# boolsi/boolsi

Measured on AMD Instinct MI355X. Metric: node-state-updates/s, higher is better.
Workload: dtype u32

## Files before the change

boolsi_amd/csrc/bsx_cascade.cpp:

```cpp
#include <cmath>
#include <cstdio>
#include <cstring>

#include "bsx_attract_host.h"

using namespace bsx;

namespace {
constexpr uint64_t kUnresCap = 1ull << 16;
constexpr uint64_t kNearBytes = 1ull << 32;
}

namespace bsx {

static int mirror_slots_for(bsx_handle h, uint32_t* slots_out) {
    const uint64_t entries = (h->cube_mirror ? 2 : 1) * h->journal_states;
    uint32_t slots = 64;
    while (slots < 2 * entries && slots < h->cache_lds_slots) slots *= 2;
    const size_t fixed = h->shmem + 32 + pool_extra_bytes(h->net.nw);
    while (slots < 4 * entries && slots < h->cache_lds_slots && fixed + (size_t)2 * slots * h->cache_stride <= 80 * 1024) slots *= 2;
    h->mirror_slots = *slots_out = std::min(slots, h->cache_lds_slots);
    if (h->knobs.debug) std::fprintf(stderr, "[bsx] mirror: %llu cycle states cached, %u slots\n", (unsigned long long)h->journal_states, *slots_out);
    return BSX_OK;
}

int lean_mirror_slots(bsx_handle h, uint32_t* slots_out, Totals* tot) {
    uint32_t ignored = 0;
    if (!slots_out) slots_out = &ignored;
    if (!h->journal_stale) return mirror_slots_for(h, slots_out);
    unsigned int known = 0;
    HIPCHK(h, hipMemcpy(&known, h->d_cc_count.p, sizeof(known), hipMemcpyDeviceToHost));
    if (tot) ++tot->syncs;
    known = std::min<unsigned int>(known, kCycleJournalCap);
    h->h_journal.resize(known);
    if (known) HIPCHK(h, hipMemcpy(h->h_journal.data(), h->d_cc_journal.p, known * sizeof(CycleRecord), hipMemcpyDeviceToHost));
    uint64_t states = 0;
    uint32_t taken = 0;
    for (const CycleRecord& r : h->h_journal) {
        if (taken >= (uint32_t)kTagAcc + kLdsAcc) break;
        if (!r.ready || r.length == 0 || r.length > kCycleCacheMaxLen) continue;
        states += r.length;
        ++taken;
    }
    h->journal_states = states;
    h->journal_stale = false;
    return mirror_slots_for(h, slots_out);
}

int ensure_mirror_image(bsx_handle h, AttractParams& P, size_t shmem) {
    if (!h->knobs.mirror_image) { P.mirror_image = nullptr; P.mirror_out = nullptr; return BSX_OK; }
    const size_t words = 4 + (size_t)P.cc.lds_slots * (h->cache_stride / 4);
    if (h->image_n != h->h_journal.size() || h->image_slots != P.cc.lds_slots || h->d_mirror.n < words) {
        HIPCHK(h, h->d_mirror.reserve(words));
        AttractParams B = P;
        B.count = 0;
        B.level_in = nullptr;
        B.mirror_image = nullptr;
        B.mirror_out = h->d_mirror.p;
        HIPCHK(h, launch_attract_pool((int)h->net.nw, (int)h->net.k_mux, h->lut_mode, dim3(1), shmem, h->stream, B));
        h->image_n = h->h_journal.size();
        h->image_slots = P.cc.lds_slots;
    }
    P.mirror_image = h->d_mirror.p;
    P.mirror_out = nullptr;
    return BSX_OK;
}

}

namespace {

int order_cube_digits(bsx_handle h, Cube& c) {
    const uint32_t r = (uint32_t)c.rel.size();
    if (r < 2 || r > 64 || !h->knobs.cube_order) return BSX_OK;
    uint64_t need = 0;
    for (uint32_t q = 0; q < r; ++q) need |= 1ull << c.rel[q];
    if (need & ~h->life_valid) {
        LifetimeParams L{};
        L.net = h->net;
        for (int w = 0; w < kMaxW32; ++w) { L.fixmask[w] = h->sp.fixmask[w]; L.fixval[w] = h->sp.fixval[w]; L.base[w] = c.base[w]; L.free_mask[w] = c.free_mask[w]; }
        L.n_digits = r;
        for (uint32_t q = 0; q < r; ++q) L.node[q] = h->model.any[c.rel[q]];
        HIPCHK(h, h->d_life.reserve(64));
        HIPCHK(h, hipMemsetAsync(h->d_life.p, 0, 64 * sizeof(uint32_t), h->stream));
        L.out = h->d_life.p;
        HIPCHK(h, launch_digit_lifetimes((int)h->net.nw, (int)h->net.k_mux, h->lut_mode, h->shmem, h->stream, L));
        uint32_t measured[64];
        HIPCHK(h, hipMemcpyAsync(measured, h->d_life.p, sizeof(measured), hipMemcpyDeviceToHost, h->stream));
        HIPCHK(h, hipStreamSynchronize(h->stream));
        for (uint32_t q = 0; q < r; ++q) h->life_cache[c.rel[q]] = measured[q];
        h->life_valid |= need;
    }
    uint32_t life[64];
    for (uint32_t q = 0; q < r; ++q) life[q] = h->life_cache[c.rel[q]];
    std::vector<uint32_t> idx(r);
    for (uint32_t q = 0; q < r; ++q) idx[q] = q;
    std::stable_sort(idx.begin(), idx.end(), [&](uint32_t x, uint32_t y) { return life[x] < life[y]; });
    std::vector<uint32_t> rel(r);
    for (uint32_t q = 0; q < r; ++q) rel[q] = c.rel[idx[q]];
    c.rel = rel;
    return BSX_OK;
}

int fetch_counters(bsx_handle h, uint32_t n_blocks) {
    if (!h->knobs.spin_wait) {
        HIPCHK(h, hipMemcpyAsync(h->h_ctr, h->d_ctr, sizeof(Counters) * n_blocks, hipMemcpyDeviceToHost, h->stream));
        HIPCHK(h, hipStreamSynchronize(h->stream));
        return BSX_OK;
    }
    const uint32_t seq = ++h->flag_seq ? h->flag_seq : ++h->flag_seq;
    HIPCHK(h, launch_publish(reinterpret_cast<const uint32_t*>(h->d_ctr), reinterpret_cast<uint32_t*>(h->h_ctr),
                             (uint32_t)(sizeof(Counters) / 4 * n_blocks), const_cast<uint32_t*>(h->h_flag), seq,
                             reinterpret_cast<unsigned int*>(reinterpret_cast<char*>(h->d_level) + kPublishTicketOffset), h->stream));
    uint32_t polls = 0;
    while (__atomic_load_n(h->h_flag, __ATOMIC_ACQUIRE) != seq) {
        __builtin_ia32_pause();
        if ((++polls & 0xFFFFu) == 0) {
            const hipError_t q = hipStreamQuery(h->stream);
            if (q == hipSuccess) {
                if (__atomic_load_n(h->h_flag, __ATOMIC_ACQUIRE) == seq) break;
                return fail(h, BSX_ERR_HIP, "the cascade finished without publishing its counters");
            }
            if (q != hipErrorNotReady) { h->error = std::string("hipStreamQuery: ") + hipGetErrorString(q); return BSX_ERR_HIP; }
        }
    }
    return BSX_OK;
}

CascadeShape cascade_shape(bsx_handle h, const CascadeEnv& env) {
    CascadeShape sh{};
    sh.tp = h->sp.tp_origin;
    sh.cap_rel = env.max_t == BSX_T_INF ? BSX_T_INF : env.max_t - sh.tp;
    sh.cap_rel32 = (sh.cap_rel == BSX_T_INF || sh.cap_rel >= (kStepLimit / 4)) ? 0xFFFFFFFFu : (uint32_t)sh.cap_rel;
    sh.fast_steps = (uint32_t)std::min<uint64_t>((uint64_t)sh.cap_rel32 + 1, std::min<uint32_t>(kFastStepsMax, std::max(192u, 4 * h->fast_steps)));
    uint32_t max_depth = h->knobs.cube_depth ? h->knobs.cube_depth : 8;
    if (h->plan.cube_depth_cap) max_depth = std::min(max_depth, h->plan.cube_depth_cap);
    if (sh.tp) max_depth = (uint32_t)std::min<uint64_t>(max_depth, sh.tp);
    sh.max_depth = std::max(1u, std::min(max_depth, sh.fast_steps > 1 ? sh.fast_steps - 1 : 1u));
    sh.forced_depth = h->knobs.cube_depth != 0;
    return sh;
}

struct ChainLevel {
    uint32_t depth = 0, k_bits = 0, r_here = 0, unit_shift = 0;
    bool per_parent = false;
    Cube cube;
};
struct Chain {
    Cube c1;
    std::vector<uint64_t> rel_mask;
    std::vector<ChainLevel> lv;
    uint32_t top = 1;
    uint32_t ctr_base = 0;
    uint32_t desc_base = 0;
    uint32_t index = 0;
    dim3 top_grid;
};
enum ChainVerdict { kChainOk = 0, kChainLower = 1, kChainRepeat = 2, kChainGiveUp = 3 };

int plan_chain(bsx_handle h, const CascadeShape& sh, const Cube& c1, uint32_t top, Chain& ch) {
    ch.c1 = c1;
    ch.lv.clear();
    cube_levels(h->model, h->sp, c1, sh.max_depth, ch.rel_mask);
    ch.top = top ? std::min<uint32_t>(top, (uint32_t)ch.rel_mask.size()) : choose_top(h->plan, sh, ch.rel_mask, sh.max_depth);
    if (__builtin_popcountll(ch.rel_mask[ch.top - 1]) > 47) return BSX_OK;
    ch.lv.resize(ch.top);
    for (uint32_t i = 0; i < ch.top; ++i) {
        const uint32_t d = ch.top - i;
        const uint64_t here = ch.rel_mask[d - 1], digits = i == 0 ? here : here & ~ch.rel_mask[d];
        ChainLevel& l = ch.lv[i];
        l.depth = d;
        l.r_here = (uint32_t)__builtin_popcountll(here);
        l.cube = c1;
        l.cube.rel.clear();
        for (uint32_t j = 0; j < c1.a; ++j) if ((digits >> j) & 1ull) l.cube.rel.push_back(j);
        if (i == 0) if (int rc = order_cube_digits(h, l.cube)) return rc;
        plan_cube(h->model, h->sp, l.cube);
        l.k_bits = (uint32_t)l.cube.rel.size();
        l.unit_shift = c1.n_free - l.r_here;
    }
    return BSX_OK;
}

struct ChainBatch {
    uint32_t slots = 0;
    size_t shmem = 0;
    Launch full{};
    uint64_t seg_cap = 0;
    uint32_t n_side = 0;
};

int prepare_batch(bsx_handle h, const CascadeEnv& env, const std::vector<Chain*>& chains, ChainBatch& B, bool& ok) {
    ok = false;
    const uint32_t nw = h->net.nw, rec_words = nw + 3;
    h->cube_mirror = true;
    const int rc_m = lean_mirror_slots(h, &B.slots, &env.tot);
    h->cube_mirror = false;
    if (rc_m) return rc_m;
    uint64_t states = 0;
    for (const CycleRecord& jr : h->h_journal) states += jr.length;
    if (h->h_journal.size() > (size_t)kTagAcc + kLdsAcc || 4 * states > h->cache_lds_slots) return BSX_OK;
    B.shmem = h->shmem + (size_t)B.slots * h->cache_stride + 32 + pool_extra_bytes(nw);
    B.full = plan_persistent(h, ~0ull >> 8, B.shmem);
    uint32_t top_bits = 16, blocks = 0;
    bool lists = false;
    for (const Chain* ch : chains) {
        if (ch->lv.empty()) continue;
        top_bits = std::max(top_bits, ch->lv[0].k_bits);
        lists = lists || ch->top > 1;
        blocks += ch->top;
    }
    const uint64_t list_cap = std::min<uint64_t>(kNearBytes / (4 * (nw + 1)), 1ull << top_bits);
    B.seg_cap = h->knobs.cube_near_cap ? h->knobs.cube_near_cap : std::max<uint64_t>(64, list_cap / B.full.grid.x);
    uint32_t n_lists = 0;
    for (const Chain* ch : chains) n_lists += (!ch->lv.empty() && ch->top > 1) ? 1u : 0u;
    B.n_side = std::min<uint32_t>(n_lists, (uint32_t)h->knobs.cube_streams);
    if (B.n_side < 2) B.n_side = lists ? 1 : 0;
    for (uint32_t sl = 0; sl < B.n_side; ++sl) {
        HIPCHK(h, h->d_near_seg[sl].reserve((size_t)B.full.grid.x * B.seg_cap * (nw + 1)));
        for (auto& list : h->d_near_list[sl]) HIPCHK(h, list.reserve((size_t)B.full.grid.x * B.seg_cap * (nw + 1)));
        if (B.n_side > 1 && !h->side[sl]) HIPCHK(h, hipStreamCreateWithFlags(&h->side[sl], hipStreamNonBlocking));
    }
    HIPCHK(h, h->d_unres.reserve((size_t)std::max(blocks, 1u) * kUnresCap * rec_words));
    ok = true;
    return BSX_OK;
}

int enqueue_chain(bsx_handle h, const CascadeEnv& env, const CascadeShape& sh, const ChainBatch& B, Chain& ch, uint32_t slot,
                  std::vector<hipEvent_t>& slot_busy) {
    const uint32_t nw = h->net.nw, rec_words = nw + 3;
    const bool side = B.n_side > 1 && ch.top > 1;
    hipStream_t const main_st = h->stream, tail_st = side ? h->side[slot] : h->stream;
    hipEvent_t* const ev = h->ev_chain.data() + 3 * (size_t)ch.index;
    if (side && slot_busy[slot]) HIPCHK(h, hipStreamWaitEvent(main_st, slot_busy[slot], 0));
    AttractParams Q0 = env.P;
    Q0.cc.lds_slots = B.slots;
    Q0.merge = 3;
    Q0.fast_steps = sh.fast_steps;
    Q0.per_problem = nullptr;
    Q0.offsets = nullptr;
    Q0.states = nullptr;
    Q0.log = nullptr; Q0.log_cap = 0; Q0.table = nullptr; Q0.table_mask = 0;
    for (int w = 0; w < kMaxW32; ++w) { Q0.cube_umask[w] = ch.c1.umask[w]; Q0.cube_free[w] = ch.c1.free_mask[w]; }
    if (int rc = ensure_mirror_image(h, Q0, B.shmem)) return rc;
    for (uint32_t i = 0; i < ch.top; ++i) {
        ChainLevel& l = ch.lv[i];
        AttractParams Q = Q0;
        Q.sp = l.cube.sp;
        Q.ctr = h->d_ctr + ch.ctr_base + i;
        Q.cube_shift = 0;
        Q.cube_depth = l.depth;
        Q.entry_shift = l.k_bits;
        Q.stragglers = h->d_unres.p + (size_t)(ch.ctr_base + i) * kUnresCap * rec_words;
        Q.stragglers_cap = kUnresCap * rec_words;
        Q.near = l.depth > 1 ? h->d_near_seg[slot].p : nullptr;
        Q.near_list = l.depth > 1 ? h->d_near_list[slot][i & 1].p : nullptr;
        Q.level_out = l.depth > 1 ? h->d_level + ch.desc_base + i + 1 : nullptr;
        Q.near_cap = l.depth > 1 ? B.seg_cap : 0;
        dim3 grid = B.full.grid;
        if (i == 0) {
            Q.count = 1ull << l.k_bits;
            Q.entries = nullptr;
            Q.level_in = nullptr;
            const Launch L = plan_persistent(h, Q.count, B.shmem);
            grid = L.grid;
            const uint64_t n_waves = (uint64_t)grid.x * (kPoolBlockThreads / 64);
            if (Q.count < (1ull << 28)) { Q.chunk_first = ((Q.count + n_waves - 1) / n_waves + 63) / 64 * 64; Q.chunk = 0; }
            else { Q.chunk_first = L.chunk; Q.chunk = L.chunk; }
            if (h->knobs.chunk) { Q.chunk = h->knobs.chunk; Q.chunk_first = Q.chunk; }
            ch.top_grid = grid;
            HIPCHK(h, hipEventRecord(ev[0], main_st));
        } else {
            Q.count = 0;
            Q.entries = h->d_near_list[slot][(i - 1) & 1].p;
            Q.level_in = h->d_level + ch.desc_base + i;
            Q.chunk = 0; Q.chunk_first = 0;
            Q.lower_build = (Q.mirror_image && h->knobs.cube_lower) ? 1u : 0u;
            if (Q.lower_build && l.depth == 1 && h->knobs.cube_leaf) {
                LeafProgram& prog = h->h_leaf[ch.index];
                if (build_leaf_program(h->model, h->sp, l.cube.rel, prog)) {
                    HIPCHK(h, hipMemcpyAsync(h->d_leaf.p + ch.index, &prog, sizeof(LeafProgram), hipMemcpyHostToDevice, tail_st));
                    Q.leaf = h->d_leaf.p + ch.index;
                    Q.entry_shift = 0;
                    l.per_parent = true;
                }
            }
        }
        const size_t shmem_here = Q.lower_build ? h->shmem + (size_t)B.slots * h->cache_stride + 32 + pool_lower_extra_bytes(nw) : B.shmem;
        hipStream_t const st = i == 0 ? main_st : tail_st;
        HIPCHK(h, launch_attract_pool((int)nw, (int)h->net.k_mux, h->lut_mode, grid, shmem_here, st, Q));
        if (i == 0) HIPCHK(h, hipEventRecord(ev[1], main_st));
        if (i == 0 && side) HIPCHK(h, hipStreamWaitEvent(tail_st, ev[1], 0));
    }
    if (side) {
        HIPCHK(h, hipEventRecord(ev[2], tail_st));
        slot_busy[slot] = ev[2];
    }
    return BSX_OK;
}

int evaluate_chain(bsx_handle h, const CascadeEnv& env, const CascadeShape& sh, const Chain& ch, MergedTable& pass_table,
                   u128& pass_none, u128& pass_ref, int& verdict, uint32_t& lower_to) {
    const AttractParams& P = env.P;
    Totals& tot = env.tot;
    const uint64_t max_t = env.max_t, max_len = env.max_len;
    const uint32_t nw = h->net.nw, rec_words = nw + 3;
    verdict = kChainOk;
    uint64_t n_entries = 0;
    for (uint32_t i = 0; i < ch.top; ++i) {
        const ChainLevel& l = ch.lv[i];
        const Counters& c = h->ctr_seen[ch.ctr_base + i];
        const uint64_t classes = i == 0 ? 1ull << l.k_bits : n_entries << l.k_bits;
        if (i > 0 && n_entries == 0) break;
        tot.steps_exec += c.steps_exec;
        if (h->knobs.debug)
            std::fprintf(stderr, "[bsx] cube 2^%u (%u digits free) at digit value %llu%s: depth %u%s, %u digits here (%u relevant), %llu classes, %llu near a cycle, %llu unresolved\n",
                         ch.c1.a, ch.c1.n_free, (unsigned long long)ch.c1.d_lo, ch.c1.fix_mask ? " [sub-block]" : "", l.depth, i == 0 ? " (top)" : l.per_parent ? " (per parent)" : "", l.k_bits, l.r_here,
                         (unsigned long long)classes, (unsigned long long)c.near_classes, (unsigned long long)c.straggler_classes);
        if (h->knobs.debug && l.per_parent) {
            const LeafProgram& prog = h->h_leaf[ch.index];
            std::fprintf(stderr, "[bsx] per-parent level: kb %u, %u enumerated rules, %u free rules, m %u\n", prog.kb, prog.n_enum, prog.n_free, prog.m);
        }
        if (c.straggler_overflow) { verdict = kChainGiveUp; return BSX_OK; }
        if (c.near_overflow) { verdict = kChainLower; lower_to = l.depth - 1; return BSX_OK; }
        n_entries = c.near_classes;
        {
            double* seen = h->plan.near_seen[i == 0 ? 0 : 1][std::min<uint32_t>(l.depth, kMaxCubeLevels)];
            seen[0] += (double)classes; seen[1] += (double)c.near_classes;
        }
        const uint32_t us = l.unit_shift;
        merge_cube_counters(pass_table, c, us, nw);
        fold_cube_level(c, us, max_t, pass_none, pass_ref);
        const uint64_t n_unres = c.straggler_classes;
        if (!n_unres) continue;
        if (n_unres > kUnresCap) { verdict = kChainGiveUp; return BSX_OK; }
        std::vector<uint32_t> recs(n_unres * rec_words);
        HIPCHK(h, hipMemcpy(recs.data(), h->d_unres.p + (size_t)(ch.ctr_base + i) * kUnresCap * rec_words, recs.size() * 4, hipMemcpyDeviceToHost));
        ++tot.syncs;
        std::vector<uint32_t> st(n_unres * nw);
        for (uint64_t q = 0; q < n_unres; ++q) std::copy(recs.begin() + q * rec_words, recs.begin() + q * rec_words + nw, st.begin() + q * nw);
        DevBuf<uint32_t> d_states;
        DevBuf<ProblemRec32> d_res;
        HIPCHK(h, d_states.upload(st));
        HIPCHK(h, d_res.alloc(n_unres));
        AttractParams S = P;
        S.sp = l.cube.sp;
        S.sp.tp_origin = 0;
        S.count = n_unres;
        S.states = d_states.p;
        S.per_problem = d_res.p;
        S.max_len = BSX_T_INF;
        S.merge = 0;
        AttractRun rs;
        if (int rc2 = launch_attract_pass(h, S, kPassGeneral, env.d_log, nullptr, rs, tot)) return rc2;
        tot.book(rs, false);
        std::vector<ProblemRec32> res(n_unres);
        HIPCHK(h, hipMemcpy(res.data(), d_res.p, n_unres * sizeof(ProblemRec32), hipMemcpyDeviceToHost));
        ++tot.syncs;
        for (uint64_t q = 0; q < n_unres; ++q)
            if (!book_unresolved_class(pass_table, pass_none, pass_ref, recs.data() + q * rec_words, res[q], nw, us, sh.tp, sh.cap_rel, max_t, max_len)) {
                verdict = kChainRepeat;
                return BSX_OK;
            }
    }
    return BSX_OK;
}

int run_batch(bsx_handle h, const CascadeEnv& env, const CascadeShape& sh, const ChainBatch& B, std::vector<Chain*>& chains) {
    Totals& tot = env.tot;
    uint32_t blocks = 0, n_live = 0;
    for (Chain* ch : chains) {
        if (ch->lv.empty()) continue;
        ch->ctr_base = blocks;
        ch->desc_base = blocks + n_live;
        ch->index = n_live++;
        blocks += ch->top;
    }
    if (!n_live) return BSX_OK;
    if (blocks > kMaxChainBlocks || n_live > kMaxChains) return fail(h, BSX_ERR_INVALID, "internal: too many chains in one batch");
    while (h->ev_chain.size() < 3 * (size_t)n_live) {
        hipEvent_t e = nullptr;
        HIPCHK(h, hipEventCreate(&e));
        h->ev_chain.push_back(e);
    }
    if (!h->h_leaf) HIPCHK(h, hipHostMalloc((void**)&h->h_leaf, sizeof(LeafProgram) * kMaxChains, hipHostMallocDefault));
    HIPCHK(h, h->d_leaf.reserve(kMaxChains));
    const double pt0 = now_ms();
    HIPCHK(h, hipMemsetAsync(h->d_level, 0, kLevelDescBytes + sizeof(Counters) * blocks, h->stream));
    HIPCHK(h, hipEventRecord(h->ev0, h->stream));
    {
        std::vector<hipEvent_t> slot_busy(std::max(1u, B.n_side), nullptr);
        uint32_t n_listing = 0;
        for (Chain* ch : chains) {
            if (ch->lv.empty()) continue;
            const uint32_t slot = (B.n_side > 1 && ch->top > 1) ? n_listing++ % B.n_side : 0u;
            if (int rc = enqueue_chain(h, env, sh, B, *ch, slot, slot_busy)) return rc;
        }
        for (hipEvent_t e : slot_busy) if (e) HIPCHK(h, hipStreamWaitEvent(h->stream, e, 0));
    }
    HIPCHK(h, hipEventRecord(h->ev1, h->stream));
    const double pt1 = now_ms();
    if (int rc = fetch_counters(h, blocks)) return rc;
    ++tot.syncs;
    const double pt2 = now_ms();
    float ms = 0.f;
    if (hipEventElapsedTime(&ms, h->ev0, h->ev1) != hipSuccess) {
        HIPCHK(h, hipEventSynchronize(h->ev1));
        HIPCHK(h, hipEventElapsedTime(&ms, h->ev0, h->ev1));
    }
    tot.prof[1] += pt1 - pt0; tot.prof[2] += pt2 - pt1; tot.prof[3] += ms;
    tot.kernel_ms += ms;
    h->ctr_seen.assign(h->h_ctr, h->h_ctr + blocks);
    for (Chain* ch : chains) {
        if (ch->lv.empty()) continue;
        float ms_top = 0.f;
        HIPCHK(h, hipEventElapsedTime(&ms_top, h->ev_chain[3 * ch->index], h->ev_chain[3 * ch->index + 1]));
        tot.launches += ch->top;
        tot.dominant_ms += ms_top;
        tot.dominant_exec += h->h_ctr[ch->ctr_base].steps_exec;
        ++tot.dominant_launches;
        if (h->knobs.debug) {
            std::string line;
            double sum = ms_top * 1e3;
            char buf[96];
            std::snprintf(buf, sizeof buf, "d%u %.0f", ch->top, ms_top * 1e3);
            line += buf;
            for (uint32_t i = 1; i < ch->top; ++i) {
                const Counters& c = h->h_ctr[ch->ctr_base + i];
                const double us = (c.t_last && c.t_first_not) ? (double)(c.t_last - ~c.t_first_not) / h->wall_clock_khz * 1e3 : 0.0;
                sum += us;
                std::snprintf(buf, sizeof buf, " | d%u %.0f", ch->top - i, us);
                line += buf;
            }
            std::fprintf(stderr, "[bsx] chain %u: estimated %.0f us, took %.0f us (%s)\n", ch->index, chain_cost_us(h->plan, ch->rel_mask, ch->top), sum, line.c_str());
        }
        for (uint32_t i = 1; i < ch->top; ++i) {
            const Counters& c = h->h_ctr[ch->ctr_base + i];
            if (!c.t_last || !c.t_first_not) continue;
            tot.lower_ms += (double)(c.t_last - ~c.t_first_not) / h->wall_clock_khz;
            tot.lower_exec += c.steps_exec;
            ++tot.lower_launches;
        }
    }
    ++tot.launches;
    return BSX_OK;
}

int run_cubes(bsx_handle h, const CascadeEnv& env, const std::vector<Cube>& cubes, bool& collapsed) {
    collapsed = false;
    Totals& tot = env.tot;
    const CascadeShape sh = cascade_shape(h, env);
    std::vector<uint32_t> top(cubes.size(), 0);
    std::vector<char> done(cubes.size(), 0);
    Totals part;
    const CascadeEnv env_part{env.P, env.max_t, env.max_len, part, env.d_log};
    auto book_device_time = [&]() {
        tot.steps_exec += part.steps_exec; tot.kernel_ms += part.kernel_ms; tot.launches += part.launches;
        tot.dominant_ms += part.dominant_ms; tot.dominant_exec += part.dominant_exec; tot.dominant_launches += part.dominant_launches;
        tot.lower_ms += part.lower_ms; tot.lower_exec += part.lower_exec; tot.lower_launches += part.lower_launches;
        tot.syncs += part.syncs; tot.limit_hits += part.limit_hits;
        for (int s = 0; s < 6; ++s) tot.prof[s] += part.prof[s];
    };
    for (int attempt = 0; attempt < 32; ++attempt) {
        const double pt_plan = now_ms();
        std::vector<Chain> chains;
        std::vector<size_t> who;
        chains.reserve(cubes.size());
        for (size_t i = 0; i < cubes.size(); ++i) {
            if (done[i]) continue;
            chains.emplace_back();
            who.push_back(i);
            if (int rc = plan_chain(h, sh, cubes[i], top[i], chains.back())) return rc;
            if (chains.back().lv.empty()) { book_device_time(); return BSX_OK; }
        }
        if (chains.empty()) break;
        std::vector<Chain*> ptrs;
        uint32_t blocks = 0;
        for (Chain& ch : chains) { ptrs.push_back(&ch); blocks += ch.top; }
        if (blocks > kMaxChainBlocks || chains.size() > kMaxChains) { book_device_time(); return BSX_OK; }
        if (ptrs.size() > 2 && h->knobs.cube_order_tails) {
            auto tail_us = [&](const Chain* ch) {
                const double top_us = kLevelOverheadUs + std::ldexp(1.0, __builtin_popcountll(ch->rel_mask[ch->top - 1])) * (ch->top + 0.3) / 4.5e5;
                return chain_cost_us(h->plan, ch->rel_mask, ch->top) - top_us;
            };
            std::vector<std::pair<double, Chain*>> keyed;
            for (Chain* ch : ptrs) keyed.emplace_back(-tail_us(ch), ch);
            std::stable_sort(keyed.begin(), keyed.end(), [](const std::pair<double, Chain*>& a, const std::pair<double, Chain*>& b) { return a.first < b.first; });
            for (size_t i = 0; i < ptrs.size(); ++i) ptrs[i] = keyed[i].second;
        }
        ChainBatch B;
        bool ok = false;
        if (int rc = prepare_batch(h, env_part, ptrs, B, ok)) return rc;
        if (!ok) { book_device_time(); return BSX_OK; }
        part.prof[0] += now_ms() - pt_plan;
        if (int rc = run_batch(h, env_part, sh, B, ptrs)) return rc;
        bool repeat = false;
        const double pt_eval = now_ms();
        for (size_t q = 0; q < chains.size(); ++q) {
            MergedTable pass_table;
            u128 pass_none = 0, pass_ref = 0;
            int verdict = kChainOk;
            uint32_t lower_to = 0;
            if (int rc = evaluate_chain(h, env_part, sh, chains[q], pass_table, pass_none, pass_ref, verdict, lower_to)) return rc;
            if (verdict == kChainOk) {
                fold_table(part.merged, pass_table);
                part.n_none += pass_none;
                part.steps_ref += pass_ref;
                done[who[q]] = 1;
            } else if (verdict == kChainLower && lower_to >= 1) {
                if (h->knobs.debug)
                    std::fprintf(stderr, "[bsx] chain %u: a list overflowed, again from depth %u\n", chains[q].index, lower_to);
                top[who[q]] = lower_to;
                if (cubes.size() == 1) h->plan.cube_depth_cap = lower_to;
            } else if (verdict == kChainRepeat) {
                repeat = true;
            } else {
                book_device_time();
                return BSX_OK;
            }
        }
        part.prof[5] += now_ms() - pt_eval;
        if (repeat) {
            unsigned int known = 0;
            HIPCHK(h, hipMemcpy(&known, h->d_cc_count.p, sizeof(known), hipMemcpyDeviceToHost));
            ++part.syncs;
            if (known <= h->h_journal.size()) { book_device_time(); return BSX_OK; }
        }
    }
    book_device_time();
    for (char d : done) if (!d) return BSX_OK;
    fold_table(tot.merged, part.merged);
    tot.n_none += part.n_none;
    tot.steps_ref += part.steps_ref;
    collapsed = true;
    return BSX_OK;
}

}

namespace bsx {

int run_block(bsx_handle h, const CascadeEnv& env, uint64_t d_lo, uint32_t a_bits, bool& collapsed) {
    collapsed = false;
    const CascadeShape sh = cascade_shape(h, env);
    const bool forced = h->knobs.cube_split == 1;
    if (h->knobs.cube_split != 0 && sh.tp == 0 && (a_bits >= kSplitMinBits || forced)) {
        std::vector<std::pair<uint64_t, uint64_t>>& tree = h->plan.split_cache[a_bits];
        auto estimate = [&]() {
            double est = 0;
            for (const auto& l : tree) est += cube_cost_us(h->model, h->sp, h->plan, sh, d_lo, a_bits, l.first, l.second);
            return est;
        };
        double experience = 0;
        for (uint32_t d = 0; d <= kMaxCubeLevels; ++d) experience += h->plan.near_seen[0][d][0];
        auto grow = [&]() {
            const double t0 = now_ms();
            std::vector<SplitLeaf> fresh;
            plan_split(h->model, h->sp, h->plan, sh, d_lo, a_bits, forced, fresh);
            tree.clear();
            for (const SplitLeaf& l : fresh) tree.emplace_back(l.mask, l.vals);
            h->plan.split_learned[a_bits] = experience;
            if (h->knobs.debug)
                std::fprintf(stderr, "[bsx] split tree for blocks of 2^%u: %zu leaves, planned in %.2f ms (list fractions from %.3g classes seen)\n", a_bits,
                             tree.size(), now_ms() - t0, experience);
        };
        const double pt_est = now_ms();
        const double whole = cube_cost_us(h->model, h->sp, h->plan, sh, d_lo, a_bits, 0, 0);
        bool use = false;
        if (tree.empty() || experience > 64.0 * (h->plan.split_learned[a_bits] + 1024.0)) { grow(); use = tree.size() > 1; }
        else if (tree.size() > 1) {
            use = forced || estimate() < 0.8 * whole;
            if (!use && a_bits >= 60 && h->plan.split_regrown[a_bits] < 2) { ++h->plan.split_regrown[a_bits]; grow(); use = tree.size() > 1; }
        }
        env.tot.prof[4] += now_ms() - pt_est;
        if (use) {
            std::vector<Cube> cubes(tree.size());
            bool eligible = true;
            for (size_t i = 0; i < tree.size() && eligible; ++i) {
                build_cube(h->model, h->sp, d_lo, a_bits, cubes[i], nullptr, tree[i].first, tree[i].second);
                if (!cubes[i].ok || cubes[i].rel.size() + 2 > cubes[i].n_free) eligible = false;
            }
            if (eligible) {
                if (int rc = run_cubes(h, env, cubes, collapsed)) return rc;
                if (collapsed) return BSX_OK;
            }
        }
    }
    Cube c;
    build_cube(h->model, h->sp, d_lo, a_bits, c);
    if (c.ok && c.rel.size() + 2 <= a_bits) return run_cubes(h, env, std::vector<Cube>{c}, collapsed);
    return BSX_OK;
}

}
```

boolsi_amd/csrc/bsx_device.h:

```cpp
#pragma once
#include <cstddef>
#include <stdint.h>

namespace bsx {

constexpr int kWave = 64;
constexpr int kBlock = 512;
constexpr int kWavesPerBlock = kBlock / kWave;
constexpr int kPoolBlockThreads = 768;
constexpr uint32_t kPoolCap = 112;
constexpr uint32_t kPoolSlots = 128;
constexpr uint32_t pool_rec_words(uint32_t nw) { return nw + 4; }
constexpr uint32_t kLowerFoundWords = 256;
constexpr int kMaxW32 = 8;
constexpr int kMaxMuxK = 6;
constexpr int kTableSlots = 64;
constexpr uint32_t kStepLimit = 1u << 30;
constexpr uint64_t kDigestSeed = 0xCBF29CE484222325ull;
constexpr uint64_t kDigestPrime = 0x100000001B3ull;
constexpr uint32_t kMaxDepositRuns = 64;

struct DevNet {
    uint32_t n_nodes;
    uint32_t nw;
    uint32_t k_mux;
    uint32_t n_chunks;
    uint32_t lut_words;
    uint32_t n_wide;
    const uint32_t* lut;
    const uint32_t* masks;
    const uint32_t* wide_desc;
    const uint32_t* wide_preds;
    const uint32_t* wide_tt;
};

struct DevSpace {
    uint32_t origin[kMaxW32];
    uint32_t fixmask[kMaxW32];
    uint32_t fixval[kMaxW32];
    uint32_t n_any;
    uint32_t identity_any;
    uint32_t n_runs;
    uint32_t deposit[2 * kMaxDepositRuns];
    uint32_t n_fv;
    uint32_t n_pv;
    uint32_t tp_origin;
    uint32_t pad;
    const uint32_t* any_nodes;
    const uint32_t* fv;
    const uint32_t* pv;
    const uint32_t* sched_set;
    const uint32_t* sched_clr;
    uint64_t first_digits[4];
    uint64_t first_variant;
};

struct LogRec {
    uint32_t key[kMaxW32];
    uint32_t length;
    uint32_t pad;
    uint64_t count;
    uint64_t sum_l;
    uint64_t sum_l2_lo, sum_l2_hi;
};
static_assert(sizeof(LogRec) == 72, "LogRec layout");

struct ProblemRec32 {
    uint32_t key[kMaxW32];
    uint32_t length;
    uint32_t trajectory_l;
    uint32_t found;
    uint32_t pad;
};

struct alignas(256) Counters {
    unsigned long long cursor;
    unsigned long long steps_ref;
    unsigned long long steps_exec;
    unsigned long long n_none;
    unsigned long long log_cursor;
    unsigned int log_overflow;
    unsigned int step_limit_hits;
    unsigned long long n_stragglers;
    unsigned long long n_cache_resolved;
    unsigned long long straggler_classes;
    unsigned int straggler_overflow;
    unsigned int pad;
    unsigned long long table_inserts;
    unsigned int table_overflow;
    unsigned int near_overflow;
    unsigned long long phase_sum[3];
    unsigned long long phase_max[3];
    unsigned long long acc_cnt[64], acc_sl[64], acc_sl2_lo[64], acc_sl2_hi[64];
    unsigned int acc_len[64];
    unsigned int acc_key[64][kMaxW32];
    unsigned long long fix_cnt[64], fix_sl[64], fix_sl2[64];
    unsigned long long fix_none, fix_ref, fix_capfail;
    unsigned long long near_classes;
    unsigned long long t_first_not, t_last;
    unsigned long long wave_iters;
    unsigned long long service_rounds;
    unsigned long long diag[4];
};

constexpr uint32_t kCycleCacheMaxLen = 64;
constexpr uint32_t kCycleCacheLdsBytes = 16 * 1024;
constexpr uint32_t kCycleJournalCap = 4096;
constexpr uint32_t kCycleClaimSlots = 8192;
constexpr int kTagAcc = 3;
constexpr uint32_t kLdsAcc = 61;
constexpr uint32_t kMergeGroup = 32;
constexpr uint32_t kMergeSlots = 256;
constexpr uint32_t lean_acc_bytes(uint32_t nw) { return (kTagAcc + kLdsAcc) * (8 + 8 + 4 + 4 + 4 * nw) + 16 + kWavesPerBlock * (kMergeSlots + 256); }

struct CycleRecord {
    uint32_t key[kMaxW32];
    uint32_t length;
    uint32_t ready;
};
static_assert(sizeof(CycleRecord) == 40, "CycleRecord layout");

struct CycleCache {
    CycleRecord* journal;
    unsigned int* journal_count;
    unsigned int* claims;
    uint32_t enabled;
    uint32_t lds_slots;
};

struct LevelDesc {
    unsigned long long n_entries;
    unsigned int abort;
    unsigned int pad;
};
constexpr uint32_t kMaxCubeLevels = 16;
constexpr uint32_t kSideStreams = 4;
constexpr uint32_t kMaxChains = 48;
constexpr uint32_t kMaxChainBlocks = 160;
constexpr size_t kLevelDescBytes = 3584;
constexpr size_t kPublishTicketOffset = kLevelDescBytes - 16;
static_assert(sizeof(LevelDesc) * (kMaxChainBlocks + kMaxChains + 1) <= kPublishTicketOffset && kLevelDescBytes % 256 == 0, "descriptor block");

constexpr uint32_t kLeafMaxDeps = 64;
constexpr uint32_t kLeafMaxBits = 14;
constexpr uint32_t kLeafMaxK = 4;
struct LeafDep {
    uint16_t in[kLeafMaxK];
    uint16_t node;
    uint16_t k;
    uint32_t tt;
};
struct LeafProgram {
    uint32_t kb, n_dep;
    uint32_t m, n_enum, n_free;
    uint32_t pad;
    uint16_t digit_node[16];
    uint32_t indep[kMaxW32];
    uint32_t added[kMaxW32];
    LeafDep dep[kLeafMaxDeps];
};

struct AttractParams {
    DevNet net;
    DevSpace sp;
    uint64_t count;
    uint32_t chunk;
    uint32_t cap_rel_inf;
    uint64_t max_t;
    uint64_t max_len;
    Counters* ctr;
    LogRec* log;
    uint64_t log_cap;
    LogRec* table;
    uint64_t table_mask;
    ProblemRec32* per_problem;
    CycleCache cc;
    const uint32_t* offsets;
    uint32_t* stragglers;
    uint64_t stragglers_cap;
    uint32_t fast_steps;
    uint32_t pad;
    uint32_t merge;
    uint32_t cube_shift;
    uint32_t cube_umask[kMaxW32];
    uint32_t cube_free[kMaxW32];
    uint32_t cube_depth;
    uint32_t entry_shift;
    const uint32_t* entries;
    uint32_t* near;
    uint32_t* near_list;
    LevelDesc* level_out;
    uint64_t near_cap;
    uint64_t chunk_first;
    const uint32_t* mirror_image;
    uint32_t* mirror_out;
    const uint32_t* states;
    const LevelDesc* level_in;
    uint32_t lower_build;
    uint32_t pad2;
    const LeafProgram* leaf;
};

constexpr uint32_t kLifeTrials = 16;
constexpr uint32_t kLifeSteps = 48;
struct LifetimeParams {
    DevNet net;
    uint32_t fixmask[kMaxW32], fixval[kMaxW32];
    uint32_t base[kMaxW32];
    uint32_t free_mask[kMaxW32];
    uint32_t n_digits;
    uint32_t pad;
    uint32_t node[64];
    uint32_t* out;
};

struct HitRec { uint64_t offset; uint64_t t; };

struct TargetParams {
    DevNet net;
    DevSpace sp;
    uint64_t count;
    uint32_t chunk;
    uint32_t cap_rel_inf;
    uint64_t max_t;
    uint32_t tmask[kMaxW32];
    uint32_t tcode[kMaxW32];
    Counters* ctr;
    uint32_t* t_hit;
    unsigned long long* hist;
    uint32_t hist_bins;
    uint32_t cube;
    uint32_t cube_shift;
    uint32_t cube_t0_shift;
    uint32_t pad;
    uint64_t chunk_first;
    uint32_t rep_mask[kMaxW32];
    uint32_t rep_code[kMaxW32];
};
constexpr uint32_t kTargetHistBins = 2048;

struct SimParams {
    DevNet net;
    DevSpace sp;
    uint64_t count;
    uint64_t max_t;
    uint32_t w64;
    uint32_t pad;
    const uint64_t* offsets;
    const uint64_t* t_len;
    const uint64_t* out_offsets;
    uint64_t* traj;
    uint64_t* final_states;
    uint64_t* digests;
    Counters* ctr;
};

constexpr int profile_block(int nw) { return nw == 8 ? 256 : kBlock; }
struct ProfileParams {
    DevNet net;
    uint32_t fixmask[kMaxW32];
    uint32_t fixval[kMaxW32];
    uint64_t count;
    uint32_t w64;
    uint32_t key_stride;
    const uint64_t* keys;
    const uint64_t* lengths;
    const uint64_t* state_offsets;
    uint32_t* on_counts;
    uint64_t* states;
    uint8_t* closed;
    Counters* ctr;
};

struct SlicedParams {
    DevSpace sp;
    uint32_t n_nodes;
    uint32_t n_rows;
    uint32_t n_sched;
    uint32_t w64;
    const uint32_t* desc;
    const uint32_t* sched;
    uint64_t count;
    uint64_t max_t;
    uint64_t* final_states;
    uint64_t* digests;
    Counters* ctr;
};

}
```

boolsi_amd/csrc/bsx_knobs.cpp:

```cpp
#include "bsx_knobs.h"

#include <algorithm>
#include <cstdlib>

#include "bsx_device.h"
#include "bsx_wide.h"

namespace bsx {

Knobs Knobs::from_env() {
    auto is_set = [](const char* name) { return std::getenv(name) != nullptr; };
    auto starts_with = [](const char* name, char c) { const char* e = std::getenv(name); return e && e[0] == c; };
    auto zero_or_one = [&](const char* name) { return starts_with(name, '0') ? 0 : starts_with(name, '1') ? 1 : -1; };
    Knobs k;
    k.debug = is_set("BSX_DEBUG");
    k.profile = is_set("BSX_PROFILE");
    k.cycle_cache = !starts_with("BSX_CYCLE_CACHE", '0');
    if (const char* e = std::getenv("BSX_CACHE_LDS_KB")) k.cache_lds_kb = std::max<size_t>(1, (size_t)std::atoi(e));
    if (const char* e = std::getenv("BSX_LUT_MODE")) k.lut_mode = std::atoi(e);
    if (const char* e = std::getenv("BSX_LEAN")) k.lean = std::atoi(e) != 0;
    if (const char* e = std::getenv("BSX_MERGE")) k.merge = std::atoi(e);
    k.force_counting = is_set("BSX_FORCE_COUNTING");
    if (const char* e = std::getenv("BSX_SERVICE_LANES")) k.service_lanes = (uint32_t)std::atoi(e);
    if (const char* e = std::getenv("BSX_CHUNK")) k.chunk = (uint32_t)std::max(64, std::atoi(e));
    k.mirror_image = !starts_with("BSX_MIRROR_IMAGE", '0');
    k.spin_wait = !starts_with("BSX_SPIN_WAIT", '0');
    k.fgraph = starts_with("BSX_FGRAPH", '1');
    k.cubes = !starts_with("BSX_CUBES", '0');
    k.cube_order = !starts_with("BSX_CUBE_ORDER", '0');
    k.cube_order_tails = !starts_with("BSX_CUBE_ORDER_TAILS", '0');
    k.cube_lower = !starts_with("BSX_CUBE_LOWER", '0');
    k.cube_leaf = !starts_with("BSX_CUBE_LEAF", '0');
    if (const char* e = std::getenv("BSX_CUBE_DEPTH")) k.cube_depth = (uint32_t)std::max(1, std::min((int)kMaxCubeLevels, std::atoi(e)));
    if (const char* e = std::getenv("BSX_CUBE_NEAR_CAP")) k.cube_near_cap = (uint64_t)std::max(1, std::atoi(e));
    const char* streams = std::getenv("BSX_CUBE_STREAMS");
    k.cube_streams = std::max(1, std::min((int)kSideStreams, streams ? std::atoi(streams) : (int)kSideStreams));
    k.cube_split = zero_or_one("BSX_CUBE_SPLIT");
    k.sliced = zero_or_one("BSX_SLICED");
    k.wide = starts_with("BSX_WIDE", '1');
    k.wide_host_reduce = starts_with("BSX_WIDE_HOST_REDUCE", '1');
    if (const char* e = std::getenv("BSX_WIDE_CHUNK")) if (e[0]) { k.wide_chunk_set = true; k.wide_chunk = std::strtoull(e, nullptr, 10); }
    k.wide_step_limit = kWideStepLimit;
    if (const char* e = std::getenv("BSX_WIDE_STEP_LIMIT")) k.wide_step_limit = std::max(16u, std::min(kWideStepLimit, (uint32_t)std::atoi(e)));
    if (const char* e = std::getenv("BSX_CORR_BATCH_CELLS")) k.corr_batch_cells = std::strtoull(e, nullptr, 10);
    k.trans_step_limit = kStepLimit;
    if (const char* e = std::getenv("BSX_TRANS_STEP_LIMIT")) k.trans_step_limit = std::max(1u, std::min(kStepLimit, (uint32_t)std::atoi(e)));
    if (const char* e = std::getenv("BSX_WTRANS_CHUNK")) k.wtrans_chunk = std::max(1ull, std::strtoull(e, nullptr, 10));
    return k;
}

}
```

boolsi_amd/csrc/bsx_knobs.h:

```cpp
#pragma once
#include <cstdint>

namespace bsx {

struct Knobs {
    bool debug = false;
    bool profile = false;
    bool cycle_cache = true;
    uint64_t cache_lds_kb = 0;
    int lut_mode = -1;
    bool lean = true;
    int merge = 2;
    bool force_counting = false;
    uint32_t service_lanes = 0;
    uint32_t chunk = 0;
    bool mirror_image = true;
    bool spin_wait = true;
    bool fgraph = false;
    bool cubes = true;
    bool cube_order = true;
    bool cube_order_tails = true;
    bool cube_lower = true;
    bool cube_leaf = true;
    uint32_t cube_depth = 0;
    uint64_t cube_near_cap = 0;
    int cube_streams = 0;
    int cube_split = -1;
    int sliced = -1;
    bool wide = false;
    bool wide_host_reduce = false;
    bool wide_chunk_set = false;
    uint64_t wide_chunk = 0;
    uint32_t wide_step_limit = 0;
    uint64_t corr_batch_cells = 0;
    uint32_t trans_step_limit = 0;
    uint64_t wtrans_chunk = 0;

    static Knobs from_env();
};

}
```

boolsi_amd/csrc/bsx_pool_kernel.h:

```cpp
#pragma once
#include "bsx_kernels_common.h"
#include "bsx_leaf.h"

namespace bsx {

constexpr int kPoolBlock = kPoolBlockThreads;
constexpr int kPoolWaves = kPoolBlock / 64;
constexpr uint32_t kPoolGroup = 64;

constexpr int pool_min_waves(int nw) { return nw <= 2 ? 6 : 2; }

#define BSX_RARE_PARAMS(name) BSX_KERNARG(AttractParams, name)

template <int NW>
__device__ __forceinline__ void deposit_runs(const DevSpace& sp, uint64_t d, uint32_t (&s)[NW], uint32_t run_first = 0,
                                             uint32_t run_end = 0xFFFFFFFFu) {
    const uint32_t end = run_end < sp.n_runs ? run_end : sp.n_runs;
    for (uint32_t r = run_first; r < end; ++r) {
        const uint32_t desc = sp.deposit[2 * r], mask = sp.deposit[2 * r + 1];
        const uint32_t piece = ((uint32_t)(d >> (desc & 63u)) & mask) << ((desc >> 16) & 31u);
        const uint32_t word = (desc >> 8) & 7u;
#pragma unroll
        for (int w = 0; w < NW; ++w) s[w] |= (word == (uint32_t)w) ? piece : 0u;
    }
}

template <int NW, int K, int LM, bool CUBE, bool LOWER = false>
__global__ __launch_bounds__(kPoolBlock, pool_min_waves(NW)) void k_attract_pool(const AttractParams P) {
    static_assert(CUBE || !LOWER, "the lower-level build is a cube build");
    extern __shared__ __attribute__((aligned(16))) uint32_t smem[];
    uint32_t* smem_free;
#ifdef BSX_DIAG
    const unsigned long long dbg_t0 = wall_clock64();
#endif
    uint64_t n_items = P.count, chunk_first = P.chunk_first;
    uint32_t chunk = P.chunk;
    if constexpr (CUBE) {
        if (P.level_in) {
            const unsigned long long listed = P.level_in->n_entries;
            n_items = P.level_in->abort ? 0ull : listed << P.entry_shift;
            if constexpr (LOWER) {
                if (P.leaf && n_items) n_items = ((listed + 63ull) & ~63ull) * leaf_parts(P.leaf->m, listed, (uint64_t)gridDim.x * kPoolWaves);
            }
            if (n_items == 0) return;
            const uint64_t n_waves = (uint64_t)gridDim.x * kPoolWaves;
            if (n_items < (1ull << 28)) { chunk_first = ((n_items + n_waves - 1) / n_waves + 63) / 64 * 64; chunk = 0; }
            else { chunk_first = 4096; chunk = 4096; }
            if ((uint64_t)blockIdx.x * chunk_first >= n_items) return;
        }
    }
    if constexpr (CUBE) {
        if (threadIdx.x == 0 && !P.mirror_out) atomicMax(&P.ctr->t_first_not, ~(unsigned long long)wall_clock64());
    }
    const NetView<NW, K, LM> nv = stage_network<NW, K, LM>(P.net, smem, smem_free);
    const uint32_t lane = threadIdx.x & 63, wave = __builtin_amdgcn_readfirstlane(threadIdx.x >> 6);
    const uint32_t tp = P.sp.tp_origin;
    const bool has_warmup = tp != 0;
    const bool counting = CUBE || P.merge >= 2;
    constexpr bool cube = CUBE;
    const int32_t fast_steps = (int32_t)P.fast_steps;
    const uint32_t cmask = P.cc.lds_slots - 1;
    constexpr int S = CacheLayout<NW>::kStride;
    constexpr uint32_t kAccs = (uint32_t)kTagAcc + kLdsAcc;
    constexpr uint32_t R = cube ? NW + 2 : pool_rec_words(NW);
    constexpr uint32_t kCap = cube ? (kPoolCap * pool_rec_words(NW)) / (NW + 2) : kPoolCap;

    uint32_t* lc = smem + (((uint32_t)(smem_free - smem) + 3u) & ~3u);
    const uint32_t lc_words = kCacheHeaderWords + P.cc.lds_slots * S;
    unsigned long long* acc_sl2 = reinterpret_cast<unsigned long long*>(lc + ((lc_words + 1u) & ~1u));
    unsigned long long* acc_sl2h = acc_sl2 + kAccs;
    unsigned long long* acc_sl = acc_sl2h + kAccs;
    unsigned long long* acc_cnt = acc_sl + kAccs;
    uint32_t* lamtab = reinterpret_cast<uint32_t*>(acc_cnt + kAccs);
    uint32_t* keytab = lamtab + kAccs;
    constexpr uint32_t kWaveWords = LOWER ? 0u : kPoolCap * pool_rec_words(NW) + 128 + kPoolSlots / 4;
    constexpr uint32_t kFoundWords = LOWER ? kLowerFoundWords : 0u;
    constexpr uint32_t kLowerCntWords = LOWER ? 2u * kAccs : 0u;
    static_assert(kAccs % 2 == 0 && kWaveWords % 2 == 0, "64-bit LDS atomics need 8-byte aligned tables");
    unsigned long long* wg_ctr = reinterpret_cast<unsigned long long*>(keytab + ((kAccs * NW + 1u) & ~1u));
    uint32_t* midtab = reinterpret_cast<uint32_t*>(wg_ctr + 4);
    uint32_t* wave_base = midtab + 64 * NW + kFoundWords + wave * (kWaveWords + kLowerCntWords);
    typedef volatile uint32_t __attribute__((address_space(3))) lds_vu32;
    typedef volatile uint8_t __attribute__((address_space(3))) lds_vu8;
    lds_vu32* const pool = (lds_vu32*)(__attribute__((address_space(3))) uint32_t*)wave_base;
    lds_vu32* const dd_acc = pool + kPoolCap * pool_rec_words(NW);
    lds_vu8* const dd_ids = (lds_vu8*)(dd_acc + 128);

    uint32_t fm0[NW], fv0[NW];
    uint32_t any_fixed = 0;
#pragma unroll
    for (int w = 0; w < NW; ++w) { fm0[w] = P.sp.fixmask[w]; fv0[w] = P.sp.fixval[w]; any_fixed |= fm0[w]; }
    const bool has_fixed = any_fixed != 0;
    const uint32_t* const image = P.mirror_image;
    if (image) { for (uint32_t i = threadIdx.x; i < lc_words; i += blockDim.x) lc[i] = image[i]; }
    else { for (uint32_t i = threadIdx.x; i < lc_words; i += blockDim.x) lc[i] = 0; }
    for (uint32_t i = threadIdx.x; i < kAccs; i += blockDim.x) { acc_sl2[i] = 0; acc_sl2h[i] = 0; acc_sl[i] = 0; acc_cnt[i] = 0; lamtab[i] = 0; }
    if (threadIdx.x < 4) wg_ctr[threadIdx.x] = 0;
    if constexpr (!LOWER) { dd_acc[2 * lane] = 0; dd_acc[2 * lane + 1] = 0; }
    else { wave_base[lane] = 0; wave_base[64 + lane] = 0; }
    __syncthreads();
    if (!image && threadIdx.x == 0) {
        uint32_t seen = 0, n_states = 0, n_attr = 0;
        cache_pull<NW, K>(P.cc, nv, fm0, fv0, lc, seen, n_states, n_attr, kAccs);
    }
    __syncthreads();
    if (P.mirror_out) {
        for (uint32_t i = threadIdx.x; i < lc_words; i += blockDim.x) P.mirror_out[i] = lc[i];
        return;
    }
    const uint32_t* cbase = lc + kCacheHeaderWords;
    for (uint32_t sl = threadIdx.x; sl < P.cc.lds_slots; sl += blockDim.x) {
        const uint32_t tg = cbase[sl * S + NW] & kTagMask;
        if (tg) {
            lamtab[tg - 1] = cbase[sl * S + NW + 1];
#pragma unroll
            for (int w = 0; w < NW; ++w) keytab[(tg - 1) * NW + w] = cbase[sl * S + NW + 2 + w];
        }
    }
    __syncthreads();
    if constexpr (cube) {
        for (uint32_t i = threadIdx.x; i < 64u; i += blockDim.x) {
            uint32_t m[NW];
#pragma unroll
            for (int w = 0; w < NW; ++w) m[w] = 0;
            deposit_runs<NW>(P.sp, (uint64_t)i << 6, m, 6u, 12u);
#pragma unroll
            for (int w = 0; w < NW; ++w) midtab[i * NW + w] = m[w];
        }
    }
    const uint32_t depth = (cube && P.cube_depth > 1u) ? P.cube_depth : 1u;
    const bool from_entries = cube && P.entries != nullptr;
    if constexpr (cube) {
        if (threadIdx.x == 0) { lc[1] = 0; lc[2] = 0; }
        __syncthreads();
        if (depth == 1u && !has_warmup) {
            constexpr uint32_t kFoundCap = LOWER ? kLowerFoundWords : kCap * R;
            auto inside = [&](uint32_t sl) -> bool {
                const uint32_t* e = cbase + sl * S;
                const uint32_t tw = e[NW];
                if ((tw & kTagMask) == 0 || (tw & kTagRep)) return false;
                uint32_t outside = 0;
#pragma unroll
                for (int w = 0; w < NW; ++w) outside |= (e[w] ^ P.sp.origin[w]) & ~P.cube_free[w];
                return outside == 0;
            };
            lds_vu32* const found0 = (lds_vu32*)(__attribute__((address_space(3))) uint32_t*)(midtab + 64 * NW);
            for (uint32_t sl = threadIdx.x; sl < P.cc.lds_slots; sl += blockDim.x) {
                if (!inside(sl)) continue;
                const uint32_t at = atomicAdd((uint32_t*)(__attribute__((address_space(3))) uint32_t*)&lc[1], 1u);
                if (at < kFoundCap) found0[at] = sl;
            }
            __syncthreads();
            if (threadIdx.x == 0) {
                const uint32_t n_in = lc[1];
                auto add_rep = [&](uint32_t sl) {
                    const uint32_t* e = cbase + sl * S;
                    uint32_t rep[NW], key[NW], differs = 0;
#pragma unroll
                    for (int w = 0; w < NW; ++w) {
                        rep[w] = e[w] & ~P.cube_umask[w];
                        differs |= rep[w] ^ e[w];
                        key[w] = e[NW + 2 + w];
                    }
                    if (differs) cache_insert_lds<NW>(lc, cmask, rep, e[NW + 1], key, (e[NW] & kTagMask) | kTagRep);
                };
                if (n_in <= kFoundCap) {
                    for (uint32_t i = 0; i < n_in; ++i) add_rep(found0[i]);
                } else {
                    for (uint32_t sl = 0; sl < P.cc.lds_slots; ++sl) if (inside(sl)) add_rep(sl);
                }
            }
        }
    }
    __syncthreads();
    const bool t0_lookup = cube && !has_warmup && depth == 1u && __builtin_amdgcn_readfirstlane(lc[1]) != 0;
    uint32_t lane_part[NW];
#pragma unroll
    for (int w = 0; w < NW; ++w) lane_part[w] = 0;
    if constexpr (cube) deposit_runs<NW>(P.sp, (uint64_t)lane, lane_part);
    uint32_t u_hi[NW];
    uint64_t u_hi_tag = ~0ull;
#pragma unroll
    for (int w = 0; w < NW; ++w) u_hi[w] = 0;

    const uint32_t cap_rel = (P.cap_rel_inf || P.max_t - tp >= (kStepLimit / 4)) ? 0xFFFFFFFFu : (uint32_t)(P.max_t - tp);

    using cnt_t = std::conditional_t<CUBE, unsigned long long, uint32_t>;
    uint32_t nexec = 0;
    const uint64_t first_dyn = (uint64_t)gridDim.x * kPoolWaves * chunk_first;
    WaveQueue q{0, 0, chunk != 0 && n_items > first_dyn};
    {
        const uint64_t b = ((uint64_t)wave * gridDim.x + blockIdx.x) * chunk_first;
        if (b < n_items) { q.next = b; q.end = (b + chunk_first < n_items) ? b + chunk_first : n_items; }
    }
    uint32_t head = 0, count = 0;
#ifdef BSX_DIAG
    unsigned long long dbg_iters = 0, dbg_fresh = 0, dbg_fresh_keep = 0, dbg_pool_in = 0, dbg_pool_keep = 0, dbg_merged = 0;
    bool dbg_is_fresh = false;
#endif

    uint32_t ptag = 0;
    auto fresh_state = [&](uint64_t pos, bool lv, uint32_t (&S0)[NW]) {
        if ((pos >> 12) != u_hi_tag) {
            u_hi_tag = pos >> 12;
#pragma unroll
            for (int w = 0; w < NW; ++w) u_hi[w] = P.sp.origin[w];
            deposit_runs<NW>(P.sp, pos & ~0xFFFull, u_hi, 12u);
        }
        const uint32_t mid = (((uint32_t)pos >> 6) & 63u) * NW;
#pragma unroll
        for (int w = 0; w < NW; ++w) S0[w] = u_hi[w] | midtab[mid + w] | lane_part[w];
        if (P.entries) {
            const uint64_t e = (pos + lane) >> P.entry_shift;
            if (lv) {
#pragma unroll
                for (int w = 0; w < NW; ++w) S0[w] |= P.entries[e * (NW + 1) + w];
                ptag = P.entries[e * (NW + 1) + NW];
            }
        }
    };

    uint32_t hit_len = 0;
    auto probe = [&](const uint32_t (&s)[NW], uint32_t& hfull, bool reps = false) -> uint32_t {
        const uint32_t ignore = reps ? 0u : kTagRep;
        hfull = hash_state<NW>(s);
        uint32_t h = hfull & cmask;
        const uint32_t* e = cbase + h * S;
        uint32_t et, d;
        if constexpr (NW == 1) {
            uint4 v = *reinterpret_cast<const uint4*>(__builtin_assume_aligned(e, 16));
            asm volatile("" : "+v"(v.w));
            d = v.x ^ s[0]; et = v.y; hit_len = v.z;
        } else if constexpr (NW == 2) {
            uint4 v = *reinterpret_cast<const uint4*>(__builtin_assume_aligned(e, 16));
            d = (v.x ^ s[0]) | (v.y ^ s[1]); et = v.z; hit_len = v.w;
        } else {
            d = 0;
#pragma unroll
            for (int w = 0; w < NW; ++w) d |= e[w] ^ s[w];
            et = e[NW];
        }
        bool hit = (d == 0) & (et != 0) & ((et & ignore) == 0);
        bool walking = (et >> 31) != 0 && !hit;
        if (__builtin_expect(__ballot(walking) != 0, 0)) {
            while (walking) {
                h = (h + 1) & cmask;
                const uint32_t* f = cbase + h * S;
                uint32_t d2 = 0;
#pragma unroll
                for (int w = 0; w < NW; ++w) d2 |= f[w] ^ s[w];
                const uint32_t ft = f[NW];
                const bool here = (d2 == 0) & (ft != 0) & ((ft & ignore) == 0);
                if (here) { hit = true; et = ft; hit_len = f[NW + 1]; }
                walking = (ft >> 31) != 0 && !here;
            }
        }
        return hit ? et : 0u;
    };

    auto account = [&](uint32_t tagw, cnt_t m, uint32_t mu, uint32_t lam, bool& keep_out) {
        const uint32_t tg = tagw & kTagMask, traj = tp + mu;
        const bool found = mu <= cap_rel && lam <= cap_rel - mu;
        const bool keep = found && (uint64_t)lam <= P.max_len;
        keep_out = keep;
        if (__builtin_expect(!keep, 0)) {
            atomicAdd(&wg_ctr[0], (unsigned long long)m);
            if (found) atomicAdd(&wg_ctr[2], (unsigned long long)m * (traj + lam));
            else atomicAdd(&wg_ctr[1], (unsigned long long)m);
        } else {
            const unsigned long long wl = (unsigned long long)m * traj;
            atomicAdd(&acc_cnt[tg - 1], (unsigned long long)m);
            atomicAdd(&acc_sl[tg - 1], wl);
            if constexpr (cube) {
                const unsigned long long lo = wl * traj, hi = __umul64hi(wl, (unsigned long long)traj);
                const unsigned long long old = atomicAdd(&acc_sl2[tg - 1], lo);
                const unsigned long long up = hi + ((old + lo < old) ? 1ull : 0ull);
                if (up) atomicAdd(&acc_sl2h[tg - 1], up);
            } else {
                atomicAdd(&acc_sl2[tg - 1], wl * traj);
            }
        }
    };

    auto account_fix = [&](uint32_t tagw, uint32_t mu, uint32_t lam, long long sign) {
        BSX_RARE_PARAMS(Pr);
        asm volatile("" : "+v"(mu));
        const uint32_t tg = tagw & kTagMask, traj = tp + mu;
        const bool found = mu <= cap_rel && lam <= cap_rel - mu;
        const bool keep = found && (uint64_t)lam <= Pr->max_len;
        Counters* c = Pr->ctr;
        if (found) atomicAdd(&c->fix_ref, (unsigned long long)(sign * (long long)(traj + lam)));
        else atomicAdd(&c->fix_capfail, (unsigned long long)sign);
        if (!keep) { atomicAdd(&c->fix_none, (unsigned long long)sign); return; }
        c->acc_len[tg - 1] = lam;
#pragma unroll
        for (int w = 0; w < NW; ++w) c->acc_key[tg - 1][w] = keytab[(tg - 1) * NW + w];
        atomicAdd(&c->fix_cnt[tg - 1], (unsigned long long)sign);
        atomicAdd(&c->fix_sl[tg - 1], (unsigned long long)(sign * (long long)traj));
        atomicAdd(&c->fix_sl2[tg - 1], (unsigned long long)(sign * (long long)traj * (long long)traj));
    };

#ifdef BSX_DIAG
    const unsigned long long dbg_t1 = wall_clock64();
#endif
    if constexpr (LOWER) {
        uint32_t* const wave_cnt = wave_base;
        if (P.leaf) {
            const LeafProgram* const L = P.leaf;
            const uint32_t kb = L->kb, n_dep = L->n_dep, m = L->m, n_enum = L->n_enum, n_free = L->n_free;
            uint32_t indep[NW], added[NW];
#pragma unroll
            for (int w = 0; w < NW; ++w) { indep[w] = L->indep[w]; added[w] = L->added[w]; }
            static_assert(sizeof(LeafDep) == 16 && kLeafMaxDeps * 4 <= kLowerFoundWords, "the rules fit the found list's words");
            uint32_t* const dep_lds = midtab + 64 * NW;
            for (uint32_t i = threadIdx.x; i < n_dep * 4u; i += blockDim.x) dep_lds[i] = reinterpret_cast<const uint32_t*>(L->dep)[i];
            __syncthreads();
            if (threadIdx.x == 0) lc[1] = 0;
            for (uint32_t sl0 = 0; sl0 < P.cc.lds_slots; sl0 += blockDim.x) {
                const uint32_t sl = sl0 + threadIdx.x;
                uint32_t ew[NW + 1];
#pragma unroll
                for (int w = 0; w <= NW; ++w) ew[w] = sl < P.cc.lds_slots ? lc[kCacheHeaderWords + sl * S + w] : 0u;
                __syncthreads();
                const bool occ = (ew[NW] & kTagMask) != 0;
                const uint64_t ob = __ballot(occ);
                uint32_t at0 = 0;
                if (lane == 0 && ob) at0 = atomicAdd((uint32_t*)(__attribute__((address_space(3))) uint32_t*)&lc[1], (uint32_t)__popcll(ob));
                const uint32_t at = __builtin_amdgcn_readfirstlane(at0) + rank_below(ob);
                if (occ) {
#pragma unroll
                    for (int w = 0; w <= NW; ++w) lc[kCacheHeaderWords + at * S + w] = ew[w];
                }
            }
            __syncthreads();
            const uint32_t n_occupied = __builtin_amdgcn_readfirstlane(lc[1]);
            const unsigned long long listed = P.level_in->n_entries, listed64 = (listed + 63ull) & ~63ull;
            const uint32_t parts = leaf_parts(m, listed, (uint64_t)gridDim.x * kPoolWaves);
            const uint32_t children_per_part = leaf_children_per_part(kb, m, parts);
            for (;;) {
                if (q.next == q.end) {
                    if (!q.more) break;
                    BSX_RARE_PARAMS(Pr);
                    const uint64_t b = first_dyn + grab_chunk(&Pr->ctr->cursor, chunk, (int)lane);
                    if (b >= n_items) { q.more = false; continue; }
                    q.next = b; q.end = (b + chunk < n_items) ? b + chunk : n_items;
                }
                const uint64_t avail = q.end - q.next;
                const uint32_t n = avail < 64u ? (uint32_t)avail : 64u;
                const uint32_t part = (uint32_t)(q.next / listed64);
                const unsigned long long pbase = q.next - (unsigned long long)part * listed64;
                const bool lv = lane < n && pbase + lane < listed;
                uint32_t Sp[NW], Y[NW], tagp = 0;
#pragma unroll
                for (int w = 0; w < NW; ++w) { Sp[w] = 0; Y[w] = 0; }
                if (lv) {
                    const uint32_t* ent = P.entries + (pbase + lane) * (NW + 1);
#pragma unroll
                    for (int w = 0; w < NW; ++w) Sp[w] = ent[w];
                    tagp = ent[NW];
                    net_step<NW, K>(nv, Sp, fm0, fv0, Y, has_fixed);
                    nexec += part == 0u ? 1u : 0u;
                }
                q.next += n;
                uint32_t hits = 0;
                for (uint32_t sl = 0; sl < n_occupied; ++sl) {
                    const uint32_t* e = cbase + sl * S;
                    const uint32_t tagw = __builtin_amdgcn_readfirstlane(e[NW]);
                    if ((tagw & kTagMask) == 0) continue;
                    {
                        uint32_t d0 = 0;
#pragma unroll
                        for (int w = 0; w < NW; ++w) d0 |= (e[w] ^ Sp[w]) & ~added[w];
                        if (lv && d0 == 0 && part == 0u) {
                            const uint32_t lam0 = lamtab[(tagw & kTagMask) - 1];
                            account_fix(tagw, 0u, lam0, 1ll);
                            account_fix(tagw, 1u, lam0, -1ll);
                        }
                        if (tagw & kTagRep) continue;
                    }
                    uint32_t d = 0;
#pragma unroll
                    for (int w = 0; w < NW; ++w) d |= (e[w] ^ Y[w]) & indep[w];
                    bool ok = lv && d == 0;
                    if (!__ballot(ok)) continue;
                    const uint32_t shift = leaf_free_shift<NW>(Sp, e, dep_lds, n_enum, n_free, kb, m);
                    ok = ok && shift != kLeafNoChild;
                    if (!__ballot(ok)) continue;
                    uint32_t n_hit = leaf_enum_hits<NW>(Sp, e, dep_lds, n_enum, m, part, parts) << (shift & 31u);
                    n_hit = ok ? n_hit : 0u;
                    if (n_hit) atomicAdd(&wave_cnt[2u * ((tagw & kTagMask) - 1u)], n_hit);
                    hits += n_hit;
                }
                if (lv) atomicAdd(&wave_cnt[2u * (tagp - 1u) + 1u], children_per_part - hits);
            }
        } else {
#ifndef BSX_LOWER_BATCHES
#define BSX_LOWER_BATCHES 2
#endif
        constexpr int B = BSX_LOWER_BATCHES;
        for (;;) {
            if (q.next == q.end) {
                if (!q.more) break;
                BSX_RARE_PARAMS(Pr);
                const uint64_t b = first_dyn + grab_chunk(&Pr->ctr->cursor, chunk, (int)lane);
                if (b >= n_items) { q.more = false; continue; }
                q.next = b; q.end = (b + chunk < n_items) ? b + chunk : n_items;
            }
            uint32_t S[B][NW], tagp[B], et[B];
            bool lv[B];
            uint64_t pos[B];
#pragma unroll
            for (int b = 0; b < B; ++b) {
                const uint64_t avail = q.end - q.next;
                const uint32_t n = avail < 64u ? (uint32_t)avail : 64u;
                lv[b] = lane < n;
                pos[b] = q.next;
#pragma unroll
                for (int w = 0; w < NW; ++w) S[b][w] = 0;
                tagp[b] = 0;
                if (n) { fresh_state(pos[b], lv[b], S[b]); tagp[b] = ptag; }
                q.next += n;
            }
            if (t0_lookup) {
#pragma unroll
                for (int b = 0; b < B; ++b) {
                    uint32_t h0;
                    const uint32_t et0 = lv[b] ? probe(S[b], h0, true) : 0u;
                    if (et0) {
                        const uint32_t lam0 = lamtab[(et0 & kTagMask) - 1];
                        bool kept;
                        uint32_t one = 1u;
                        unsigned long long m0 = 1ull << P.cube_shift;
                        asm volatile("" : "+v"(one), "+v"(m0));
                        account(et0, m0, one, lam0, kept);
                        account_fix(et0, 0u, lam0, 1ll);
                        account_fix(et0, 1u, lam0, -1ll);
                        lv[b] = false;
                    }
                }
            }
            for (uint32_t i = 1; i < depth; ++i) {
#pragma unroll
                for (int b = 0; b < B; ++b) {
                    if (lv[b]) {
                        uint32_t nx[NW];
                        net_step<NW, K>(nv, S[b], fm0, fv0, nx, has_fixed);
#pragma unroll
                        for (int w = 0; w < NW; ++w) S[b][w] = nx[w];
                    }
                }
            }
#pragma unroll
            for (int b = 0; b < B; ++b) {
                et[b] = 0;
                if (lv[b]) {
                    uint32_t nx[NW], hf;
                    net_step<NW, K>(nv, S[b], fm0, fv0, nx, has_fixed);
                    et[b] = probe(nx, hf);
                    nexec += depth;
                }
            }
#pragma unroll
            for (int b = 0; b < B; ++b) {
                if (depth > 1u) {
                    const bool near = lv[b] && et[b] != 0;
                    const uint64_t nb = __ballot(near);
                    if (nb) {
                        BSX_RARE_PARAMS(Pr);
                        uint32_t S0[NW];
                        fresh_state(pos[b], near, S0);
                        uint32_t at0 = 0;
                        if (lane == 0) at0 = atomicAdd((uint32_t*)(__attribute__((address_space(3))) uint32_t*)&lc[2], (uint32_t)__popcll(nb));
                        const uint32_t at = __builtin_amdgcn_readfirstlane(at0) + rank_below(nb);
                        if (near && at < Pr->near_cap) {
                            uint32_t* seg = Pr->near + ((uint64_t)blockIdx.x * Pr->near_cap + at) * (NW + 1);
#pragma unroll
                            for (int w = 0; w < NW; ++w) seg[w] = S0[w];
                            seg[NW] = et[b] & kTagMask;
                        }
                    }
                    if (near) lv[b] = false;
                }
                const bool hit = lv[b] && et[b] != 0;
                const uint32_t otag = hit ? (et[b] & kTagMask) : tagp[b];
                bool todo = lv[b];
                uint64_t tb = __ballot(todo);
                while (tb) {
                    const int first = __builtin_ctzll(tb);
                    const uint32_t tg = (uint32_t)__builtin_amdgcn_readlane((int)otag, first);
                    const bool h0 = __builtin_amdgcn_readlane((int)(hit ? 1u : 0u), first) != 0;
                    const bool same = todo && otag == tg && hit == h0;
                    const uint64_t sb = __ballot(same);
                    if (lane == (uint32_t)first) atomicAdd(&wave_cnt[2u * (tg - 1u) + (h0 ? 0u : 1u)], (uint32_t)__popcll(sb));
                    todo = todo && !same;
                    tb &= ~sb;
                }
            }
        }
        }
        __builtin_amdgcn_fence(__ATOMIC_ACQ_REL, "wavefront");
        __builtin_amdgcn_wave_barrier();
#pragma unroll
        for (uint32_t half = 0; half < 2; ++half) {
            const uint32_t idx = half * 64u + lane;
            const uint32_t n_classes = *(volatile uint32_t*)&wave_cnt[idx];
            if (n_classes) {
                const uint32_t tg = idx / 2u + 1u;
                bool kept;
                account(tg, (cnt_t)(((unsigned long long)n_classes) << P.cube_shift), depth + (idx & 1u), lamtab[tg - 1], kept);
            }
        }
    }
    if constexpr (!LOWER) for (;;) {
        const bool input = q.more || q.next < q.end;
        if (!input && count == 0) break;
#ifdef BSX_DIAG
        ++dbg_iters;
#endif
        uint32_t A[NW], base = 0, mlo = 0, mhi = 0, res = 0, hfull = 0;
        int32_t t = 0;
        bool live = false, deep_fresh = false;
        uint64_t fresh_pos = 0;
        if (count > kCap - kPoolGroup || !input) {
            const uint32_t n = count < 64u ? count : 64u;
            live = lane < n;
            uint32_t ri = head + lane;
            ri -= ri >= kCap ? kCap : 0u;
            const uint32_t r = ri * R;
            if constexpr (cube) {
                uint32_t packed;
                if constexpr (NW == 2) {
                    typedef volatile bsx_u32x4 __attribute__((address_space(3))) lds_v4;
                    const bsx_u32x4 v = *(lds_v4*)(pool + r);
                    A[0] = live ? v.x : 0u; A[1] = live ? v.y : 0u; mlo = v.z; packed = v.w;
                } else {
#pragma unroll
                    for (int w = 0; w < NW; ++w) A[w] = live ? pool[r + w] : 0u;
                    mlo = pool[r + NW]; packed = pool[r + NW + 1];
                }
                mhi = packed & 0x1FFFFu;
                t = (int32_t)(packed >> 17) - 256;
            } else if constexpr (NW % 2 == 0) {
                typedef volatile bsx_u32x2 __attribute__((address_space(3))) lds_v2;
                lds_v2* rec = (lds_v2*)(pool + r);
#pragma unroll
                for (int w = 0; w < NW; w += 2) { const bsx_u32x2 v = rec[w / 2]; A[w] = live ? v.x : 0u; A[w + 1] = live ? v.y : 0u; }
                const bsx_u32x2 b0 = rec[NW / 2], b1 = rec[NW / 2 + 1];
                base = b0.x; mlo = b0.y; mhi = b1.x; t = (int32_t)b1.y;
            } else {
#pragma unroll
                for (int w = 0; w < NW; ++w) A[w] = live ? pool[r + w] : 0u;
                base = pool[r + NW]; mlo = pool[r + NW + 1]; mhi = pool[r + NW + 2]; t = (int32_t)pool[r + NW + 3];
            }
            head += n;
            head -= head >= kCap ? kCap : 0u;
            count -= n;
#ifdef BSX_DIAG
            dbg_is_fresh = false;
            dbg_pool_in += n;
#endif
        } else {
            if (q.next == q.end) {
                BSX_RARE_PARAMS(Pr);
                const uint64_t b = first_dyn + grab_chunk(&Pr->ctr->cursor, chunk, (int)lane);
                if (b >= n_items) { q.more = false; continue; }
                q.next = b; q.end = (b + chunk < n_items) ? b + chunk : n_items;
            }
            const uint64_t avail = q.end - q.next;
            const uint32_t n = avail < 64u ? (uint32_t)avail : 64u;
            live = lane < n;
            base = (uint32_t)q.next;
            if constexpr (cube) {
                fresh_pos = q.next;
                fresh_state(fresh_pos, live, A);
            } else {
                uint32_t lane_here = lane;
                asm volatile("" : "+v"(lane_here));
                init_problem_simple<NW>(P.sp, q.next + lane_here, A);
            }
            if (counting) {
                const unsigned long long members = 1ull << (cube ? P.cube_shift : 0u);
                mlo = (uint32_t)members; mhi = (uint32_t)(members >> 32);
            } else {
                mlo = lane < 32u ? 1u << lane : 0u;
                mhi = lane < 32u ? 0u : 1u << (lane - 32u);
            }
            t = -(int32_t)tp;
            q.next += n;
            if constexpr (cube) {
                if (t0_lookup) {
                    uint32_t h0;
                    const uint32_t et0 = live ? probe(A, h0, true) : 0u;
                    if (et0) {
                        const uint32_t lam0 = NW <= 2 ? hit_len : lamtab[(et0 & kTagMask) - 1];
                        bool kept;
                        uint32_t one = 1u;
                        unsigned long long m0 = ((unsigned long long)mhi << 32) | mlo;
                        asm volatile("" : "+v"(one), "+v"(m0));
                        account(et0, m0, one, lam0, kept);
                        account_fix(et0, 0u, lam0, 1ll);
                        account_fix(et0, 1u, lam0, -1ll);
                        live = false;
                    }
                }
            }
            if constexpr (cube) {
                if (depth > 1u) {
                    deep_fresh = !has_warmup;
                    for (uint32_t i = 1; i < depth; ++i) {
                        ++t;
                        if (live) {
                            uint32_t nx[NW];
                            net_step<NW, K>(nv, A, fm0, fv0, nx, has_fixed);
                            if (has_warmup) apply_perturbations<NW>(P.sp, (uint32_t)((int32_t)tp + t), 0ull, nx);
#pragma unroll
                            for (int w = 0; w < NW; ++w) A[w] = nx[w];
                        }
                    }
                    if (live) nexec += depth - 1u;
                }
            }
#ifdef BSX_DIAG
            ++dbg_fresh;
            dbg_is_fresh = true;
#endif
        }

        if (live && res == 0) {
            uint32_t nxt[NW];
            net_step<NW, K>(nv, A, fm0, fv0, nxt, has_fixed);
            ++t;
            ++nexec;
            if (has_warmup) {
                if (t <= 0) apply_perturbations<NW>(P.sp, (uint32_t)((int32_t)tp + t), 0ull, nxt);
            }
            uint32_t et = probe(nxt, hfull);
            if (has_warmup) et = t >= 0 ? et : 0u;
            if (!has_warmup && !cube && __ballot(et != 0 && t == 1)) {
                if (et != 0 && t == 1) {
                    uint32_t h0;
                    const uint32_t len1 = hit_len;
                    const uint32_t et0 = probe(A, h0);
                    if (et0) { et = et0; t = 0; } else hit_len = len1;
                }
            }
#pragma unroll
            for (int w = 0; w < NW; ++w) A[w] = nxt[w];
            res = et;
        }
        if constexpr (cube) {
            if (deep_fresh) {
                const bool near = live && res != 0;
                const uint64_t nb = __ballot(near);
                if (nb) {
                    BSX_RARE_PARAMS(Pr);
                    uint32_t S0[NW];
                    fresh_state(fresh_pos, near, S0);
                    uint32_t at0 = 0;
                    if (lane == 0) at0 = atomicAdd((uint32_t*)(__attribute__((address_space(3))) uint32_t*)&lc[2], (uint32_t)__popcll(nb));
                    const uint32_t at = __builtin_amdgcn_readfirstlane(at0) + rank_below(nb);
                    if (near && at < Pr->near_cap) {
                        uint32_t* seg = Pr->near + ((uint64_t)blockIdx.x * Pr->near_cap + at) * (NW + 1);
#pragma unroll
                        for (int w = 0; w < NW; ++w) seg[w] = S0[w];
                        seg[NW] = res & kTagMask;
                    }
                }
                if (near) { live = false; res = 0; }
            }
            if (from_entries) {
                const bool hit = live && res != 0;
                uint32_t otag = hit ? (res & kTagMask) : ptag;
                bool todo = live;
                uint64_t tb = __ballot(todo);
                while (tb) {
                    const int first = __builtin_ctzll(tb);
                    const uint32_t tg = (uint32_t)__builtin_amdgcn_readlane((int)otag, first);
                    const bool h0 = __builtin_amdgcn_readlane((int)(hit ? 1u : 0u), first) != 0;
                    const bool same = todo && otag == tg && hit == h0;
                    const uint64_t sb = __ballot(same);
                    if (lane == (uint32_t)first) {
                        bool kept;
                        account(tg, (cnt_t)((((unsigned long long)mhi << 32) | mlo) * (unsigned long long)__popcll(sb)),
                                (uint32_t)t + (h0 ? 0u : 1u), lamtab[tg - 1], kept);
                    }
                    todo = todo && !same;
                    tb &= ~sb;
                }
                continue;
            }
        }

        bool cand = live && res == 0 && t < fast_steps;
        uint32_t slot;
        if constexpr (cube) {
            slot = (__umul24(hfull ^ (uint32_t)t, 0x9E3779u) >> 17) & (kPoolSlots - 1);
        } else {
            const uint32_t hx = hfull ^ (hfull >> 15) ^ (counting ? (uint32_t)t : base >> 6);
            slot = ((__umul24(hx, 0x9E3779u) ^ __umul24(hx >> 11, 0x85EBCBu)) >> 12) & (kPoolSlots - 1);
        }
        if (cand) dd_ids[slot] = (uint8_t)lane;
        __builtin_amdgcn_fence(__ATOMIC_RELEASE, "wavefront");
        __builtin_amdgcn_wave_barrier();
        const uint32_t w = cand ? (uint32_t)dd_ids[slot] : lane;

        cnt_t m;
        if constexpr (cube) m = ((unsigned long long)mhi << 32) | mlo;
        else m = counting ? mlo : (uint32_t)(__popc(mlo) + __popc(mhi));
        if (live && res != 0) {
            const uint32_t tg = res & kTagMask;
            const uint32_t lam = NW <= 2 ? hit_len : lamtab[tg - 1];
            bool keep;
            account(res, m, (uint32_t)t, lam, keep);
            if (!cube && P.per_problem) {
                ProblemRec32 r;
#pragma unroll
                for (int w = 0; w < kMaxW32; ++w) r.key[w] = 0;
                if (keep) {
#pragma unroll
                    for (int w = 0; w < NW; ++w) r.key[w] = keytab[(tg - 1) * NW + w];
                }
                r.length = keep ? lam : 0; r.trajectory_l = keep ? tp + (uint32_t)t : 0; r.found = keep; r.pad = 0;
                for (uint32_t left = mlo; left; left &= left - 1) P.per_problem[base + (uint32_t)__builtin_ctz(left)] = r;
                for (uint32_t left = mhi; left; left &= left - 1) P.per_problem[base + 32u + (uint32_t)__builtin_ctz(left)] = r;
            }
        }
        if (live && res == 0 && t >= fast_steps) {
            BSX_RARE_PARAMS(Pr);
            Counters* const c = Pr->ctr;
            uint32_t* const list = Pr->stragglers;
            const uint64_t list_cap = Pr->stragglers_cap;
            if (counting && !cube) atomicOr(&c->straggler_overflow, 2u);
            atomicAdd(&c->n_stragglers, (unsigned long long)m);
            const unsigned long long at = atomicAdd(&c->straggler_classes, 1ull);
            if (cube) {
                constexpr uint32_t kRec = NW + 3;
                if (kRec * (at + 1) <= list_cap) {
#pragma unroll
                    for (int w = 0; w < NW; ++w) list[kRec * at + w] = A[w];
                    list[kRec * at + NW] = (uint32_t)t; list[kRec * at + NW + 1] = mlo; list[kRec * at + NW + 2] = mhi;
                } else atomicOr(&c->straggler_overflow, 1u);
            } else if (3 * at + 2 < list_cap) { list[3 * at] = base; list[3 * at + 1] = mlo; list[3 * at + 2] = mhi; }
            else atomicOr(&c->straggler_overflow, 1u);
        }

        {
            uint32_t differ = counting ? 0u : (uint32_t)__builtin_amdgcn_ds_bpermute((int)(w * 4u), (int)base) ^ base;
            const uint32_t tc = ((uint32_t)t << 1) | (cand ? 0u : 1u);
            differ |= (uint32_t)__builtin_amdgcn_ds_bpermute((int)(w * 4u), (int)tc) ^ ((uint32_t)t << 1);
#pragma unroll
            for (int i = 0; i < NW; ++i) differ |= (uint32_t)__builtin_amdgcn_ds_bpermute((int)(w * 4u), (int)A[i]) ^ A[i];
            const bool same = cand & (w != lane) & (differ == 0u);
#ifdef BSX_DIAG
            dbg_merged += __popcll(__ballot(same));
#endif
            if (__ballot(same)) {
                if (same) {
                    if constexpr (cube) {
                        atomicAdd((unsigned long long*)(__attribute__((address_space(3))) unsigned long long*)&dd_acc[2 * w],
                                  ((unsigned long long)mhi << 32) | mlo);
                    } else if (counting) {
                        atomicAdd((uint32_t*)(__attribute__((address_space(3))) uint32_t*)&dd_acc[2 * w], mlo);
                    } else {
                        if (mlo) atomicOr((uint32_t*)(__attribute__((address_space(3))) uint32_t*)&dd_acc[2 * w], mlo);
                        if (mhi) atomicOr((uint32_t*)(__attribute__((address_space(3))) uint32_t*)&dd_acc[2 * w + 1], mhi);
                    }
                    cand = false;
                }
                __builtin_amdgcn_fence(__ATOMIC_RELEASE, "wavefront");
                __builtin_amdgcn_wave_barrier();
                if (cand) {
                    uint32_t glo, ghi;
                    if constexpr (cube) {
                        typedef volatile bsx_u32x2 __attribute__((address_space(3))) lds_v2;
                        const bsx_u32x2 gv = *(lds_v2*)(dd_acc + 2 * lane);
                        glo = gv.x; ghi = gv.y;
                    } else { glo = dd_acc[2 * lane]; ghi = dd_acc[2 * lane + 1]; }
                    if (glo | ghi) {
                        if constexpr (cube) {
                            const unsigned long long sum = (((unsigned long long)mhi << 32) | mlo) + (((unsigned long long)ghi << 32) | glo);
                            mlo = (uint32_t)sum; mhi = (uint32_t)(sum >> 32);
                        } else if (counting) { mlo += glo; }
                        else { mlo |= glo; mhi |= ghi; }
                        dd_acc[2 * lane] = 0; dd_acc[2 * lane + 1] = 0;
                    }
                }
            }
        }

        const uint64_t keepers = __ballot(cand);
#ifdef BSX_DIAG
        if (dbg_is_fresh) dbg_fresh_keep += __popcll(keepers); else dbg_pool_keep += __popcll(keepers);
#endif
        if (cand) {
            const uint32_t rank = rank_below(keepers);
            uint32_t tail = head + count;
            tail -= tail >= kCap ? kCap : 0u;
            uint32_t ri = tail + rank;
            ri -= ri >= kCap ? kCap : 0u;
            const uint32_t r = ri * R;
            if constexpr (cube) {
                const uint32_t packed = mhi | ((uint32_t)(t + 256) << 17);
                if constexpr (NW == 2) {
                    typedef volatile bsx_u32x4 __attribute__((address_space(3))) lds_v4;
                    bsx_u32x4 v;
                    v.x = A[0]; v.y = A[1]; v.z = mlo; v.w = packed;
                    *(lds_v4*)(pool + r) = v;
                } else {
#pragma unroll
                    for (int w = 0; w < NW; ++w) pool[r + w] = A[w];
                    pool[r + NW] = mlo; pool[r + NW + 1] = packed;
                }
            } else if constexpr (NW % 2 == 0) {
                typedef volatile bsx_u32x2 __attribute__((address_space(3))) lds_v2;
                lds_v2* rec = (lds_v2*)(pool + r);
#pragma unroll
                for (int w = 0; w < NW; w += 2) { bsx_u32x2 v; v.x = A[w]; v.y = A[w + 1]; rec[w / 2] = v; }
                bsx_u32x2 b0, b1;
                b0.x = base; b0.y = mlo; b1.x = mhi; b1.y = (uint32_t)t;
                rec[NW / 2] = b0; rec[NW / 2 + 1] = b1;
            } else {
#pragma unroll
                for (int w = 0; w < NW; ++w) pool[r + w] = A[w];
                pool[r + NW] = base; pool[r + NW + 1] = mlo; pool[r + NW + 2] = mhi; pool[r + NW + 3] = (uint32_t)t;
            }
        }
        count += (uint32_t)__popcll(keepers);
        __builtin_amdgcn_fence(__ATOMIC_RELEASE, "wavefront");
        __builtin_amdgcn_wave_barrier();
    }

    __syncthreads();
#ifdef BSX_DIAG
    const unsigned long long dbg_t2 = wall_clock64();
#endif
    static_assert(kAccs == 64, "one lane per accumulator");
    if (wave == 0) {
        const uint32_t a = lane;
        const unsigned long long cn = acc_cnt[a];
        const uint64_t nb = __ballot(cn != 0);
        if (nb) {
            unsigned long long at0 = 0;
            if (!cube && lane == 0) at0 = atomicAdd(&P.ctr->log_cursor, (unsigned long long)__popcll(nb));
            const unsigned long long at = bcast64(at0, 0) + rank_below(nb);
            if (cn) {
                const unsigned long long sl = acc_sl[a];
                if constexpr (cube) {
                    Counters* c = P.ctr;
                    atomicAdd(&c->acc_cnt[a], cn);
                    atomicAdd(&c->acc_sl[a], sl);
                    const unsigned long long lo = acc_sl2[a];
                    const unsigned long long old = atomicAdd(&c->acc_sl2_lo[a], lo);
                    const unsigned long long up = acc_sl2h[a] + ((old + lo < old) ? 1ull : 0ull);
                    if (up) atomicAdd(&c->acc_sl2_hi[a], up);
                    c->acc_len[a] = lamtab[a];
#pragma unroll
                    for (int w = 0; w < NW; ++w) c->acc_key[a][w] = keytab[a * NW + w];
                } else if (at < P.log_cap) {
                    LogRec r;
#pragma unroll
                    for (int w = 0; w < kMaxW32; ++w) r.key[w] = 0;
#pragma unroll
                    for (int w = 0; w < NW; ++w) r.key[w] = keytab[a * NW + w];
                    r.length = lamtab[a]; r.pad = 0; r.count = cn; r.sum_l = sl; r.sum_l2_lo = acc_sl2[a]; r.sum_l2_hi = acc_sl2h[a];
                    P.log[at] = r;
                } else {
                    atomicOr(&P.ctr->log_overflow, 1u);
                }
                atomicAdd(&wg_ctr[2], sl + cn * lamtab[a]);
            }
        }
    }
#ifdef BSX_DIAG
    if (lane == 0) {
        atomicAdd(&P.ctr->wave_iters, dbg_iters); atomicAdd(&P.ctr->service_rounds, dbg_fresh);
        atomicAdd(&P.ctr->diag[0], dbg_fresh_keep); atomicAdd(&P.ctr->diag[1], dbg_pool_in);
        atomicAdd(&P.ctr->diag[2], dbg_pool_keep); atomicAdd(&P.ctr->diag[3], dbg_merged);
    }
    if (threadIdx.x == 0) {
        const unsigned long long dbg_t3 = wall_clock64();
        atomicAdd(&P.ctr->phase_sum[0], dbg_t1 - dbg_t0); atomicMax(&P.ctr->phase_max[0], dbg_t1 - dbg_t0);
        atomicAdd(&P.ctr->phase_sum[1], dbg_t2 - dbg_t1); atomicMax(&P.ctr->phase_max[1], dbg_t2 - dbg_t1);
        atomicAdd(&P.ctr->phase_sum[2], dbg_t3 - dbg_t2); atomicMax(&P.ctr->phase_max[2], dbg_t3 - dbg_t2);
    }
#endif
    {
        const unsigned long long w_exec = wave_sum((unsigned long long)nexec);
        if (lane == 0 && w_exec) atomicAdd(&wg_ctr[3], w_exec);
    }
    __builtin_amdgcn_fence(__ATOMIC_RELEASE, "workgroup");
    __builtin_amdgcn_s_barrier();
    __builtin_amdgcn_fence(__ATOMIC_ACQUIRE, "workgroup");
    if (threadIdx.x == 0) {
        if constexpr (cube) {
            BSX_RARE_PARAMS(Pr);
            if (Pr->level_out) {
                const uint32_t listed = lc[2];
                const uint32_t mine = listed < Pr->near_cap ? listed : (uint32_t)Pr->near_cap;
                lc[1] = mine ? (uint32_t)atomicAdd(&Pr->level_out->n_entries, (unsigned long long)mine) : 0u;
                if (listed) atomicAdd(&P.ctr->near_classes, (unsigned long long)listed);
                if (listed > Pr->near_cap) {
                    atomicOr(&Pr->level_out->abort, 1u);
                    atomicOr(&P.ctr->near_overflow, 1u);
                }
            }
        }
        const unsigned long long ref = wg_ctr[2] + (P.cap_rel_inf ? 0ull : wg_ctr[1] * P.max_t);
        if (ref) atomicAdd(&P.ctr->steps_ref, ref);
        if (wg_ctr[3]) atomicAdd(&P.ctr->steps_exec, wg_ctr[3]);
        if (wg_ctr[0]) atomicAdd(&P.ctr->n_none, wg_ctr[0]);
        if constexpr (cube) atomicMax(&P.ctr->t_last, (unsigned long long)wall_clock64());
    }
    if constexpr (cube) {
        BSX_RARE_PARAMS(Pr);
        if (Pr->level_out) {
            __syncthreads();
            const uint32_t listed = lc[2], base = lc[1];
            const uint64_t words = (uint64_t)(listed < Pr->near_cap ? listed : (uint32_t)Pr->near_cap) * (NW + 1);
            const uint32_t* src = Pr->near + (uint64_t)blockIdx.x * Pr->near_cap * (NW + 1);
            uint32_t* dst = Pr->near_list + (uint64_t)base * (NW + 1);
            for (uint64_t i = threadIdx.x; i < words; i += kPoolBlock) dst[i] = src[i];
        }
    }
}

template <int NW, int K, int LM>
__global__ __launch_bounds__(1024) void k_digit_lifetimes(const LifetimeParams P) {
    extern __shared__ __attribute__((aligned(16))) uint32_t smem[];
    uint32_t* smem_free;
    const NetView<NW, K, LM> nv = stage_network<NW, K, LM>(P.net, smem, smem_free);
    const uint32_t digit = threadIdx.x / kLifeTrials, trial = threadIdx.x % kLifeTrials;
    if (digit >= P.n_digits) return;
    uint32_t fm[NW], fv[NW], x[NW], y[NW];
    uint32_t any_fixed = 0;
    const uint32_t node = P.node[digit];
#pragma unroll
    for (int w = 0; w < NW; ++w) {
        fm[w] = P.fixmask[w]; fv[w] = P.fixval[w]; any_fixed |= fm[w];
        uint32_t rnd = (trial * 0x9E3779B1u + (uint32_t)w * 0x85EBCA6Bu + 0x27D4EB2Fu) * 0xC2B2AE35u;
        rnd ^= rnd >> 15; rnd *= 0x2C1B3C6Du; rnd ^= rnd >> 12;
        const uint32_t bit = ((node >> 5) == (uint32_t)w) ? 1u << (node & 31) : 0u;
        x[w] = (P.base[w] | (trial ? rnd & P.free_mask[w] : 0u)) & ~bit;
        y[w] = x[w] | bit;
    }
    uint32_t t = 0;
    while (t < kLifeSteps && !eq_words<NW>(x, y)) {
        uint32_t nx[NW], ny[NW];
        net_step<NW, K>(nv, x, fm, fv, nx, any_fixed != 0);
        net_step<NW, K>(nv, y, fm, fv, ny, any_fixed != 0);
        copy_words<NW>(x, nx); copy_words<NW>(y, ny);
        ++t;
    }
    atomicAdd(&P.out[digit], t);
}


template <int NW, int K>
static hipError_t launch_life_nk(int lut_mode, dim3, size_t shmem, hipStream_t st, const LifetimeParams& P) {
    const void* fn;
    BSX_KERNEL_FOR_MODE(k_digit_lifetimes, NW, K, lut_mode, fn);
    if (!fn) return hipErrorInvalidValue;
    hipError_t e = hipFuncSetAttribute(fn, hipFuncAttributeMaxDynamicSharedMemorySize, (int)shmem);
    if (e != hipSuccess) return e;
    void* args[] = {const_cast<LifetimeParams*>(&P)};
    return hipLaunchKernel(fn, dim3(1), dim3(1024), args, shmem, st);
}

template <int NW, int K>
static const void* pool_kernel_for(int lut_mode, bool cube, bool lower = false) {
    const void* fn = nullptr;
    if (lower) {
        if (lut_mode == kLutLdsByte) fn = (const void*)k_attract_pool<NW, K, kLutLdsByte, true, true>;
        else if (lut_mode == kLutGlobal) fn = (const void*)k_attract_pool<NW, K, kLutGlobal, true, true>;
        else if constexpr (NW >= 4) { if (lut_mode == kLutLdsNibble) fn = (const void*)k_attract_pool<NW, K, kLutLdsNibble, true, true>; }
    } else if (cube) {
        if (lut_mode == kLutLdsByte) fn = (const void*)k_attract_pool<NW, K, kLutLdsByte, true>;
        else if (lut_mode == kLutGlobal) fn = (const void*)k_attract_pool<NW, K, kLutGlobal, true>;
        else if constexpr (NW >= 4) { if (lut_mode == kLutLdsNibble) fn = (const void*)k_attract_pool<NW, K, kLutLdsNibble, true>; }
    } else {
        if (lut_mode == kLutLdsByte) fn = (const void*)k_attract_pool<NW, K, kLutLdsByte, false>;
        else if (lut_mode == kLutGlobal) fn = (const void*)k_attract_pool<NW, K, kLutGlobal, false>;
        else if constexpr (NW >= 4) { if (lut_mode == kLutLdsNibble) fn = (const void*)k_attract_pool<NW, K, kLutLdsNibble, false>; }
    }
    return fn;
}
template <int NW, int K>
static hipError_t launch_pool_nk(int lut_mode, dim3 grid, size_t shmem, hipStream_t st, const AttractParams& P) {
    const void* fn = pool_kernel_for<NW, K>(lut_mode, P.merge == 3, P.merge == 3 && P.lower_build != 0);
    if (!fn) return hipErrorInvalidValue;
    void* args[] = {const_cast<AttractParams*>(&P)};
    return hipLaunchKernel(fn, grid, dim3(kPoolBlock), args, shmem, st);
}
template <int NW, int K>
static hipError_t configure_pool_nk(int lut_mode, dim3, size_t shmem, hipStream_t, int& blocks_per_cu) {
    for (int cube = 0; cube < 3; ++cube) {
        const void* fn = pool_kernel_for<NW, K>(lut_mode, cube != 0, cube == 2);
        if (!fn) return hipErrorInvalidValue;
        hipError_t e = hipFuncSetAttribute(fn, hipFuncAttributeMaxDynamicSharedMemorySize, (int)shmem);
        if (e != hipSuccess) return e;
        if (!cube) { e = hipOccupancyMaxActiveBlocksPerMultiprocessor(&blocks_per_cu, fn, kPoolBlock, shmem); if (e != hipSuccess) return e; }
    }
    return hipSuccess;
}

}

#ifndef BSX_POOL_KMASK
#define BSX_POOL_KMASK 0x7E
#endif
#if BSX_POOL_KMASK & (1 << 1)
#define BSX_PK1(FN, NWV) case 1: return FN<NWV, 1>(lut_mode, grid, shmem, st, P);
#else
#define BSX_PK1(FN, NWV)
#endif
#if BSX_POOL_KMASK & (1 << 2)
#define BSX_PK2(FN, NWV) case 2: return FN<NWV, 2>(lut_mode, grid, shmem, st, P);
#else
#define BSX_PK2(FN, NWV)
#endif
#if BSX_POOL_KMASK & (1 << 3)
#define BSX_PK3(FN, NWV) case 3: return FN<NWV, 3>(lut_mode, grid, shmem, st, P);
#else
#define BSX_PK3(FN, NWV)
#endif
#if BSX_POOL_KMASK & (1 << 4)
#define BSX_PK4(FN, NWV) case 4: return FN<NWV, 4>(lut_mode, grid, shmem, st, P);
#else
#define BSX_PK4(FN, NWV)
#endif
#if BSX_POOL_KMASK & (1 << 5)
#define BSX_PK5(FN, NWV) case 5: return FN<NWV, 5>(lut_mode, grid, shmem, st, P);
#else
#define BSX_PK5(FN, NWV)
#endif
#if BSX_POOL_KMASK & (1 << 6)
#define BSX_PK6(FN, NWV) case 6: return FN<NWV, 6>(lut_mode, grid, shmem, st, P);
#else
#define BSX_PK6(FN, NWV)
#endif
#define BSX_POOL_DISPATCH_K(FN, NWV)                                                                                  \
    switch (k) {                                                                                                      \
        BSX_PK1(FN, NWV) BSX_PK2(FN, NWV) BSX_PK3(FN, NWV) BSX_PK4(FN, NWV) BSX_PK5(FN, NWV) BSX_PK6(FN, NWV)          \
        default: return hipErrorInvalidValue;                                                                         \
    }

#define BSX_POOL_TU(NWV, TAG)                                                                                         \
    namespace bsx {                                                                                                   \
    hipError_t launch_pool_nw##NWV##TAG(int k, int lut_mode, dim3 grid, size_t shmem, hipStream_t st, const AttractParams& P) { \
        BSX_POOL_DISPATCH_K(launch_pool_nk, NWV)                                                                      \
    }                                                                                                                 \
    hipError_t configure_pool_nw##NWV##TAG(int k, int lut_mode, size_t shmem, int* blocks_per_cu) {                   \
        const dim3 grid(1);                                                                                           \
        const hipStream_t st = nullptr;                                                                               \
        int& P = *blocks_per_cu;                                                                                      \
        BSX_POOL_DISPATCH_K(configure_pool_nk, NWV)                                                                   \
    }                                                                                                                 \
    hipError_t launch_life_nw##NWV##TAG(int k, int lut_mode, size_t shmem, hipStream_t st, const LifetimeParams& P) { \
        const dim3 grid(1);                                                                                           \
        BSX_POOL_DISPATCH_K(launch_life_nk, NWV)                                                                      \
    }                                                                                                                 \
    }
```

Baseline: 16480 billion.

## Fuse the per-parent leaf level into the depth-2 cube launch

When the chain's next level is a depth-1 leaf, the depth-2 launch now runs the leaf per-parent enumeration in the same kernel, using the near-cycle entries it just produced. This removes one kernel launch per chain along with the global near-list round trip and copy between the two levels. The fused kernel books leaf counters into the next counter slot, and the host accounting is adjusted to match. It adds complexity to the work split inside one launch, and changes how the leaf work is divided across waves.

After: 16520 billion (median of 3 runs). No clear change (+0.2%).

```diff
diff --git a/boolsi_amd/csrc/bsx_cascade.cpp b/boolsi_amd/csrc/bsx_cascade.cpp
--- a/boolsi_amd/csrc/bsx_cascade.cpp
+++ b/boolsi_amd/csrc/bsx_cascade.cpp
@@ -144,6 +144,7 @@
 struct ChainLevel {
     uint32_t depth = 0, k_bits = 0, r_here = 0, unit_shift = 0;
     bool per_parent = false;
+    bool fused = false;
     Cube cube;
 };
 struct Chain {
@@ -238,6 +239,7 @@
     Q0.merge = 3;
     Q0.fast_steps = sh.fast_steps;
     Q0.per_problem = nullptr;
+    Q0.leaf = nullptr; Q0.leaf_fused = 0;
     Q0.offsets = nullptr;
     Q0.states = nullptr;
     Q0.log = nullptr; Q0.log_cap = 0; Q0.table = nullptr; Q0.table_mask = 0;
@@ -276,13 +278,17 @@
             Q.level_in = h->d_level + ch.desc_base + i;
             Q.chunk = 0; Q.chunk_first = 0;
             Q.lower_build = (Q.mirror_image && h->knobs.cube_lower) ? 1u : 0u;
-            if (Q.lower_build && l.depth == 1 && h->knobs.cube_leaf) {
+            const bool leaf_here = l.depth == 1, leaf_below = l.depth == 2 && h->knobs.cube_leaf_fused;
+            if (Q.lower_build && (leaf_here || leaf_below) && h->knobs.cube_leaf) {
+                ChainLevel& leaf = leaf_here ? l : ch.lv[i + 1];
                 LeafProgram& prog = h->h_leaf[ch.index];
-                if (build_leaf_program(h->model, h->sp, l.cube.rel, prog)) {
+                if (build_leaf_program(h->model, h->sp, leaf.cube.rel, prog)) {
                     HIPCHK(h, hipMemcpyAsync(h->d_leaf.p + ch.index, &prog, sizeof(LeafProgram), hipMemcpyHostToDevice, tail_st));
                     Q.leaf = h->d_leaf.p + ch.index;
-                    Q.entry_shift = 0;
-                    l.per_parent = true;
+                    if (leaf_here) Q.entry_shift = 0;
+                    else Q.leaf_fused = 1u;
+                    leaf.per_parent = true;
+                    leaf.fused = leaf_below;
                 }
             }
         }
@@ -291,6 +297,7 @@
         HIPCHK(h, launch_attract_pool((int)nw, (int)h->net.k_mux, h->lut_mode, grid, shmem_here, st, Q));
         if (i == 0) HIPCHK(h, hipEventRecord(ev[1], main_st));
         if (i == 0 && side) HIPCHK(h, hipStreamWaitEvent(tail_st, ev[1], 0));
+        if (Q.leaf_fused) break;
     }
     if (side) {
         HIPCHK(h, hipEventRecord(ev[2], tail_st));
@@ -315,14 +322,18 @@
         tot.steps_exec += c.steps_exec;
         if (h->knobs.debug)
             std::fprintf(stderr, "[bsx] cube 2^%u (%u digits free) at digit value %llu%s: depth %u%s, %u digits here (%u relevant), %llu classes, %llu near a cycle, %llu unresolved\n",
-                         ch.c1.a, ch.c1.n_free, (unsigned long long)ch.c1.d_lo, ch.c1.fix_mask ? " [sub-block]" : "", l.depth, i == 0 ? " (top)" : l.per_parent ? " (per parent)" : "", l.k_bits, l.r_here,
+                         ch.c1.a, ch.c1.n_free, (unsigned long long)ch.c1.d_lo, ch.c1.fix_mask ? " [sub-block]" : "", l.depth, i == 0 ? " (top)" : l.fused ? " (per parent, fused)" : l.per_parent ? " (per parent)" : "", l.k_bits, l.r_here,
                          (unsigned long long)classes, (unsigned long long)c.near_classes, (unsigned long long)c.straggler_classes);
         if (h->knobs.debug && l.per_parent) {
             const LeafProgram& prog = h->h_leaf[ch.index];
             std::fprintf(stderr, "[bsx] per-parent level: kb %u, %u enumerated rules, %u free rules, m %u\n", prog.kb, prog.n_enum, prog.n_free, prog.m);
         }
         if (c.straggler_overflow) { verdict = kChainGiveUp; return BSX_OK; }
-        if (c.near_overflow) { verdict = kChainLower; lower_to = l.depth - 1; return BSX_OK; }
+        if (c.near_overflow) {
+            if (i + 1 < ch.top && ch.lv[i + 1].fused) tot.steps_exec += h->ctr_seen[ch.ctr_base + i + 1].steps_exec;
+            verdict = kChainLower; lower_to = l.depth - 1;
+            return BSX_OK;
+        }
         n_entries = c.near_classes;
         {
             double* seen = h->plan.near_seen[i == 0 ? 0 : 1][std::min<uint32_t>(l.depth, kMaxCubeLevels)];
@@ -415,7 +426,7 @@
         if (ch->lv.empty()) continue;
         float ms_top = 0.f;
         HIPCHK(h, hipEventElapsedTime(&ms_top, h->ev_chain[3 * ch->index], h->ev_chain[3 * ch->index + 1]));
-        tot.launches += ch->top;
+        tot.launches += ch->top - (ch->lv.back().fused ? 1u : 0u);
         tot.dominant_ms += ms_top;
         tot.dominant_exec += h->h_ctr[ch->ctr_base].steps_exec;
         ++tot.dominant_launches;
@@ -429,13 +440,15 @@
                 const Counters& c = h->h_ctr[ch->ctr_base + i];
                 const double us = (c.t_last && c.t_first_not) ? (double)(c.t_last - ~c.t_first_not) / h->wall_clock_khz * 1e3 : 0.0;
                 sum += us;
-                std::snprintf(buf, sizeof buf, " | d%u %.0f", ch->top - i, us);
+                if (ch->lv[i].fused) std::snprintf(buf, sizeof buf, " | d%u fused", ch->top - i);
+                else std::snprintf(buf, sizeof buf, " | d%u %.0f", ch->top - i, us);
                 line += buf;
             }
             std::fprintf(stderr, "[bsx] chain %u: estimated %.0f us, took %.0f us (%s)\n", ch->index, chain_cost_us(h->plan, ch->rel_mask, ch->top), sum, line.c_str());
         }
         for (uint32_t i = 1; i < ch->top; ++i) {
             const Counters& c = h->h_ctr[ch->ctr_base + i];
+            if (ch->lv[i].fused) { tot.lower_exec += c.steps_exec; continue; }
             if (!c.t_last || !c.t_first_not) continue;
             tot.lower_ms += (double)(c.t_last - ~c.t_first_not) / h->wall_clock_khz;
             tot.lower_exec += c.steps_exec;
diff --git a/boolsi_amd/csrc/bsx_device.h b/boolsi_amd/csrc/bsx_device.h
--- a/boolsi_amd/csrc/bsx_device.h
+++ b/boolsi_amd/csrc/bsx_device.h
@@ -197,7 +197,7 @@
     const uint32_t* states;
     const LevelDesc* level_in;
     uint32_t lower_build;
-    uint32_t pad2;
+    uint32_t leaf_fused;
     const LeafProgram* leaf;
 };
 
diff --git a/boolsi_amd/csrc/bsx_knobs.cpp b/boolsi_amd/csrc/bsx_knobs.cpp
--- a/boolsi_amd/csrc/bsx_knobs.cpp
+++ b/boolsi_amd/csrc/bsx_knobs.cpp
@@ -31,6 +31,7 @@
     k.cube_order_tails = !starts_with("BSX_CUBE_ORDER_TAILS", '0');
     k.cube_lower = !starts_with("BSX_CUBE_LOWER", '0');
     k.cube_leaf = !starts_with("BSX_CUBE_LEAF", '0');
+    k.cube_leaf_fused = !starts_with("BSX_CUBE_LEAF_FUSED", '0');
     if (const char* e = std::getenv("BSX_CUBE_DEPTH")) k.cube_depth = (uint32_t)std::max(1, std::min((int)kMaxCubeLevels, std::atoi(e)));
     if (const char* e = std::getenv("BSX_CUBE_NEAR_CAP")) k.cube_near_cap = (uint64_t)std::max(1, std::atoi(e));
     const char* streams = std::getenv("BSX_CUBE_STREAMS");
diff --git a/boolsi_amd/csrc/bsx_knobs.h b/boolsi_amd/csrc/bsx_knobs.h
--- a/boolsi_amd/csrc/bsx_knobs.h
+++ b/boolsi_amd/csrc/bsx_knobs.h
@@ -22,6 +22,7 @@
     bool cube_order_tails = true;
     bool cube_lower = true;
     bool cube_leaf = true;
+    bool cube_leaf_fused = true;
     uint32_t cube_depth = 0;
     uint64_t cube_near_cap = 0;
     int cube_streams = 0;
diff --git a/boolsi_amd/csrc/bsx_pool_kernel.h b/boolsi_amd/csrc/bsx_pool_kernel.h
--- a/boolsi_amd/csrc/bsx_pool_kernel.h
+++ b/boolsi_amd/csrc/bsx_pool_kernel.h
@@ -40,7 +40,7 @@
             const unsigned long long listed = P.level_in->n_entries;
             n_items = P.level_in->abort ? 0ull : listed << P.entry_shift;
             if constexpr (LOWER) {
-                if (P.leaf && n_items) n_items = ((listed + 63ull) & ~63ull) * leaf_parts(P.leaf->m, listed, (uint64_t)gridDim.x * kPoolWaves);
+                if (P.leaf && !P.leaf_fused && n_items) n_items = ((listed + 63ull) & ~63ull) * leaf_parts(P.leaf->m, listed, (uint64_t)gridDim.x * kPoolWaves);
             }
             if (n_items == 0) return;
             const uint64_t n_waves = (uint64_t)gridDim.x * kPoolWaves;
@@ -130,10 +130,12 @@
     }
     const uint32_t depth = (cube && P.cube_depth > 1u) ? P.cube_depth : 1u;
     const bool from_entries = cube && P.entries != nullptr;
+    bool fused_leaf = false;
+    if constexpr (LOWER) fused_leaf = P.leaf != nullptr && P.leaf_fused != 0u;
     if constexpr (cube) {
         if (threadIdx.x == 0) { lc[1] = 0; lc[2] = 0; }
         __syncthreads();
-        if (depth == 1u && !has_warmup) {
+        if ((depth == 1u || fused_leaf) && !has_warmup) {
             constexpr uint32_t kFoundCap = LOWER ? kLowerFoundWords : kCap * R;
             auto inside = [&](uint32_t sl) -> bool {
                 const uint32_t* e = cbase + sl * S;
@@ -282,13 +284,14 @@
         }
     };
 
+    uint32_t ctr_off = 0;
     auto account_fix = [&](uint32_t tagw, uint32_t mu, uint32_t lam, long long sign) {
         BSX_RARE_PARAMS(Pr);
         asm volatile("" : "+v"(mu));
         const uint32_t tg = tagw & kTagMask, traj = tp + mu;
         const bool found = mu <= cap_rel && lam <= cap_rel - mu;
         const bool keep = found && (uint64_t)lam <= Pr->max_len;
-        Counters* c = Pr->ctr;
+        Counters* c = Pr->ctr + ctr_off;
         if (found) atomicAdd(&c->fix_ref, (unsigned long long)(sign * (long long)(traj + lam)));
         else atomicAdd(&c->fix_capfail, (unsigned long long)sign);
         if (!keep) { atomicAdd(&c->fix_none, (unsigned long long)sign); return; }
@@ -303,97 +306,112 @@
 #ifdef BSX_DIAG
     const unsigned long long dbg_t1 = wall_clock64();
 #endif
+    auto flush_sums = [&](Counters* const c) {
+        __syncthreads();
+#ifdef BSX_DIAG
+        const unsigned long long dbg_t2 = wall_clock64();
+#endif
+        static_assert(kAccs == 64, "one lane per accumulator");
+        if (wave == 0) {
+            const uint32_t a = lane;
+            const unsigned long long cn = acc_cnt[a];
+            const uint64_t nb = __ballot(cn != 0);
+            if (nb) {
+                unsigned long long at0 = 0;
+                if (!cube && lane == 0) at0 = atomicAdd(&c->log_cursor, (unsigned long long)__popcll(nb));
+                const unsigned long long at = bcast64(at0, 0) + rank_below(nb);
+                if (cn) {
+                    const unsigned long long sl = acc_sl[a];
+                    if constexpr (cube) {
+                        atomicAdd(&c->acc_cnt[a], cn);
+                        atomicAdd(&c->acc_sl[a], sl);
+                        const unsigned long long lo = acc_sl2[a];
+                        const unsigned long long old = atomicAdd(&c->acc_sl2_lo[a], lo);
+                        const unsigned long long up = acc_sl2h[a] + ((old + lo < old) ? 1ull : 0ull);
+                        if (up) atomicAdd(&c->acc_sl2_hi[a], up);
+                        c->acc_len[a] = lamtab[a];
+#pragma unroll
+                        for (int w = 0; w < NW; ++w) c->acc_key[a][w] = keytab[a * NW + w];
+                    } else if (at < P.log_cap) {
+                        LogRec r;
+#pragma unroll
+                        for (int w = 0; w < kMaxW32; ++w) r.key[w] = 0;
+#pragma unroll
+                        for (int w = 0; w < NW; ++w) r.key[w] = keytab[a * NW + w];
+                        r.length = lamtab[a]; r.pad = 0; r.count = cn; r.sum_l = sl; r.sum_l2_lo = acc_sl2[a]; r.sum_l2_hi = acc_sl2h[a];
+                        P.log[at] = r;
+                    } else {
+                        atomicOr(&c->log_overflow, 1u);
+                    }
+                    atomicAdd(&wg_ctr[2], sl + cn * lamtab[a]);
+                }
+            }
+        }
+#ifdef BSX_DIAG
+        if (c == P.ctr) {
+            if (lane == 0) {
+                atomicAdd(&c->wave_iters, dbg_iters); atomicAdd(&c->service_rounds, dbg_fresh);
+                atomicAdd(&c->diag[0], dbg_fresh_keep); atomicAdd(&c->diag[1], dbg_pool_in);
+                atomicAdd(&c->diag[2], dbg_pool_keep); atomicAdd(&c->diag[3], dbg_merged);
+            }
+            if (threadIdx.x == 0) {
+                const unsigned long long dbg_t3 = wall_clock64();
+                atomicAdd(&c->phase_sum[0], dbg_t1 - dbg_t0); atomicMax(&c->phase_max[0], dbg_t1 - dbg_t0);
+                atomicAdd(&c->phase_sum[1], dbg_t2 - dbg_t1); atomicMax(&c->phase_max[1], dbg_t2 - dbg_t1);
+                atomicAdd(&c->phase_sum[2], dbg_t3 - dbg_t2); atomicMax(&c->phase_max[2], dbg_t3 - dbg_t2);
+            }
+        }
+#endif
+        {
+            const unsigned long long w_exec = wave_sum((unsigned long long)nexec);
+            if (lane == 0 && w_exec) atomicAdd(&wg_ctr[3], w_exec);
+        }
+        __builtin_amdgcn_fence(__ATOMIC_RELEASE, "workgroup");
+        __builtin_amdgcn_s_barrier();
+        __builtin_amdgcn_fence(__ATOMIC_ACQUIRE, "workgroup");
+    };
+    auto note_listed = [&](bool reserve) {
+        BSX_RARE_PARAMS(Pr);
+        if (Pr->level_out) {
+            const uint32_t listed = lc[2];
+            const uint32_t mine = listed < Pr->near_cap ? listed : (uint32_t)Pr->near_cap;
+            if (reserve) lc[1] = mine ? (uint32_t)atomicAdd(&Pr->level_out->n_entries, (unsigned long long)mine) : 0u;
+            if (listed) atomicAdd(&P.ctr->near_classes, (unsigned long long)listed);
+            if (listed > Pr->near_cap) {
+                atomicOr(&Pr->level_out->abort, 1u);
+                atomicOr(&P.ctr->near_overflow, 1u);
+            }
+        }
+    };
+    auto flush_ctrs = [&](Counters* const c) {
+        const unsigned long long ref = wg_ctr[2] + (P.cap_rel_inf ? 0ull : wg_ctr[1] * P.max_t);
+        if (ref) atomicAdd(&c->steps_ref, ref);
+        if (wg_ctr[3]) atomicAdd(&c->steps_exec, wg_ctr[3]);
+        if (wg_ctr[0]) atomicAdd(&c->n_none, wg_ctr[0]);
+    };
     if constexpr (LOWER) {
         uint32_t* const wave_cnt = wave_base;
-        if (P.leaf) {
-            const LeafProgram* const L = P.leaf;
-            const uint32_t kb = L->kb, n_dep = L->n_dep, m = L->m, n_enum = L->n_enum, n_free = L->n_free;
-            uint32_t indep[NW], added[NW];
-#pragma unroll
-            for (int w = 0; w < NW; ++w) { indep[w] = L->indep[w]; added[w] = L->added[w]; }
-            static_assert(sizeof(LeafDep) == 16 && kLeafMaxDeps * 4 <= kLowerFoundWords, "the rules fit the found list's words");
-            uint32_t* const dep_lds = midtab + 64 * NW;
-            for (uint32_t i = threadIdx.x; i < n_dep * 4u; i += blockDim.x) dep_lds[i] = reinterpret_cast<const uint32_t*>(L->dep)[i];
-            __syncthreads();
-            if (threadIdx.x == 0) lc[1] = 0;
-            for (uint32_t sl0 = 0; sl0 < P.cc.lds_slots; sl0 += blockDim.x) {
-                const uint32_t sl = sl0 + threadIdx.x;
-                uint32_t ew[NW + 1];
-#pragma unroll
-                for (int w = 0; w <= NW; ++w) ew[w] = sl < P.cc.lds_slots ? lc[kCacheHeaderWords + sl * S + w] : 0u;
-                __syncthreads();
-                const bool occ = (ew[NW] & kTagMask) != 0;
-                const uint64_t ob = __ballot(occ);
-                uint32_t at0 = 0;
-                if (lane == 0 && ob) at0 = atomicAdd((uint32_t*)(__attribute__((address_space(3))) uint32_t*)&lc[1], (uint32_t)__popcll(ob));
-                const uint32_t at = __builtin_amdgcn_readfirstlane(at0) + rank_below(ob);
-                if (occ) {
-#pragma unroll
-                    for (int w = 0; w <= NW; ++w) lc[kCacheHeaderWords + at * S + w] = ew[w];
-                }
-            }
-            __syncthreads();
-            const uint32_t n_occupied = __builtin_amdgcn_readfirstlane(lc[1]);
-            const unsigned long long listed = P.level_in->n_entries, listed64 = (listed + 63ull) & ~63ull;
-            const uint32_t parts = leaf_parts(m, listed, (uint64_t)gridDim.x * kPoolWaves);
-            const uint32_t children_per_part = leaf_children_per_part(kb, m, parts);
-            for (;;) {
-                if (q.next == q.end) {
-                    if (!q.more) break;
-                    BSX_RARE_PARAMS(Pr);
-                    const uint64_t b = first_dyn + grab_chunk(&Pr->ctr->cursor, chunk, (int)lane);
-                    if (b >= n_items) { q.more = false; continue; }
-                    q.next = b; q.end = (b + chunk < n_items) ? b + chunk : n_items;
-                }
-                const uint64_t avail = q.end - q.next;
-                const uint32_t n = avail < 64u ? (uint32_t)avail : 64u;
-                const uint32_t part = (uint32_t)(q.next / listed64);
-                const unsigned long long pbase = q.next - (unsigned long long)part * listed64;
-                const bool lv = lane < n && pbase + lane < listed;
-                uint32_t Sp[NW], Y[NW], tagp = 0;
-#pragma unroll
-                for (int w = 0; w < NW; ++w) { Sp[w] = 0; Y[w] = 0; }
-                if (lv) {
-                    const uint32_t* ent = P.entries + (pbase + lane) * (NW + 1);
-#pragma unroll
-                    for (int w = 0; w < NW; ++w) Sp[w] = ent[w];
-                    tagp = ent[NW];
-                    net_step<NW, K>(nv, Sp, fm0, fv0, Y, has_fixed);
-                    nexec += part == 0u ? 1u : 0u;
-                }
-                q.next += n;
-                uint32_t hits = 0;
-                for (uint32_t sl = 0; sl < n_occupied; ++sl) {
-                    const uint32_t* e = cbase + sl * S;
-                    const uint32_t tagw = __builtin_amdgcn_readfirstlane(e[NW]);
-                    if ((tagw & kTagMask) == 0) continue;
-                    {
-                        uint32_t d0 = 0;
-#pragma unroll
-                        for (int w = 0; w < NW; ++w) d0 |= (e[w] ^ Sp[w]) & ~added[w];
-                        if (lv && d0 == 0 && part == 0u) {
-                            const uint32_t lam0 = lamtab[(tagw & kTagMask) - 1];
-                            account_fix(tagw, 0u, lam0, 1ll);
-                            account_fix(tagw, 1u, lam0, -1ll);
-                        }
-                        if (tagw & kTagRep) continue;
-                    }
-                    uint32_t d = 0;
-#pragma unroll
-                    for (int w = 0; w < NW; ++w) d |= (e[w] ^ Y[w]) & indep[w];
-                    bool ok = lv && d == 0;
-                    if (!__ballot(ok)) continue;
-                    const uint32_t shift = leaf_free_shift<NW>(Sp, e, dep_lds, n_enum, n_free, kb, m);
-                    ok = ok && shift != kLeafNoChild;
-                    if (!__ballot(ok)) continue;
-                    uint32_t n_hit = leaf_enum_hits<NW>(Sp, e, dep_lds, n_enum, m, part, parts) << (shift & 31u);
-                    n_hit = ok ? n_hit : 0u;
-                    if (n_hit) atomicAdd(&wave_cnt[2u * ((tagw & kTagMask) - 1u)], n_hit);
-                    hits += n_hit;
-                }
-                if (lv) atomicAdd(&wave_cnt[2u * (tagp - 1u) + 1u], children_per_part - hits);
-            }
-        } else {
+        auto book_outcomes = [&](uint32_t dep) {
+            __builtin_amdgcn_fence(__ATOMIC_ACQ_REL, "wavefront");
+            __builtin_amdgcn_wave_barrier();
+#pragma unroll
+            for (uint32_t half = 0; half < 2; ++half) {
+                const uint32_t idx = half * 64u + lane;
+                const uint32_t n_classes = *(volatile uint32_t*)&wave_cnt[idx];
+                if (n_classes) {
+                    const uint32_t tg = idx / 2u + 1u;
+                    bool kept;
+                    account(tg, (cnt_t)(((unsigned long long)n_classes) << P.cube_shift), dep + (idx & 1u), lamtab[tg - 1], kept);
+                }
+            }
+        };
+        const LeafProgram* L = fused_leaf ? nullptr : P.leaf;
+        const uint32_t* parents = P.entries;
+        unsigned long long listed = L ? P.level_in->n_entries : 0ull;
+        uint64_t leaf_waves = (uint64_t)gridDim.x * kPoolWaves, leaf_share = (uint64_t)wave * gridDim.x + blockIdx.x;
+        bool own_segment = false;
+        uint32_t book_depth = depth;
+        if (!L) {
 #ifndef BSX_LOWER_BATCHES
 #define BSX_LOWER_BATCHES 2
 #endif
@@ -498,18 +516,132 @@
             }
         }
         }
-        __builtin_amdgcn_fence(__ATOMIC_ACQ_REL, "wavefront");
-        __builtin_amdgcn_wave_barrier();
-#pragma unroll
-        for (uint32_t half = 0; half < 2; ++half) {
-            const uint32_t idx = half * 64u + lane;
-            const uint32_t n_classes = *(volatile uint32_t*)&wave_cnt[idx];
-            if (n_classes) {
-                const uint32_t tg = idx / 2u + 1u;
-                bool kept;
-                account(tg, (cnt_t)(((unsigned long long)n_classes) << P.cube_shift), depth + (idx & 1u), lamtab[tg - 1], kept);
-            }
-        }
+        if (fused_leaf) {
+            BSX_RARE_PARAMS(Pr);
+            book_outcomes(depth);
+            flush_sums(P.ctr);
+            if (threadIdx.x == 0) { note_listed(false); flush_ctrs(P.ctr); }
+            auto uniform64 = [](uint64_t v) -> uint64_t {
+                return ((uint64_t)(uint32_t)__builtin_amdgcn_readfirstlane((int)(uint32_t)(v >> 32)) << 32) | (uint32_t)__builtin_amdgcn_readfirstlane((int)(uint32_t)v);
+            };
+            const uint32_t n_listed = (uint32_t)__builtin_amdgcn_readfirstlane((int)lc[2]);
+            const uint64_t seg_cap = uniform64(Pr->near_cap);
+            if (n_listed == 0u || n_listed > seg_cap) {
+                if (threadIdx.x == 0) atomicMax(&P.ctr->t_last, (unsigned long long)wall_clock64());
+                return;
+            }
+            __syncthreads();
+            for (uint32_t i = threadIdx.x; i < kAccs; i += blockDim.x) { acc_sl2[i] = 0; acc_sl2h[i] = 0; acc_sl[i] = 0; acc_cnt[i] = 0; }
+            if (threadIdx.x < 4) wg_ctr[threadIdx.x] = 0;
+            wave_cnt[lane] = 0; wave_cnt[64 + lane] = 0;
+            nexec = 0;
+            L = P.leaf;
+            parents = (const uint32_t*)uniform64((uint64_t)Pr->near) + (uint64_t)blockIdx.x * seg_cap * (NW + 1);
+            listed = n_listed;
+            leaf_waves = kPoolWaves; leaf_share = wave;
+            own_segment = true;
+            book_depth = 1u;
+            ctr_off = 1u;
+        }
+        if (L) {
+            const uint32_t kb = L->kb, n_dep = L->n_dep, m = L->m, n_enum = L->n_enum, n_free = L->n_free;
+            uint32_t indep[NW], added[NW];
+#pragma unroll
+            for (int w = 0; w < NW; ++w) { indep[w] = L->indep[w]; added[w] = L->added[w]; }
+            static_assert(sizeof(LeafDep) == 16 && kLeafMaxDeps * 4 <= kLowerFoundWords, "the rules fit the found list's words");
+            uint32_t* const dep_lds = midtab + 64 * NW;
+            for (uint32_t i = threadIdx.x; i < n_dep * 4u; i += blockDim.x) dep_lds[i] = reinterpret_cast<const uint32_t*>(L->dep)[i];
+            __syncthreads();
+            if (threadIdx.x == 0) lc[1] = 0;
+            for (uint32_t sl0 = 0; sl0 < P.cc.lds_slots; sl0 += blockDim.x) {
+                const uint32_t sl = sl0 + threadIdx.x;
+                uint32_t ew[NW + 1];
+#pragma unroll
+                for (int w = 0; w <= NW; ++w) ew[w] = sl < P.cc.lds_slots ? lc[kCacheHeaderWords + sl * S + w] : 0u;
+                __syncthreads();
+                const bool occ = (ew[NW] & kTagMask) != 0;
+                const uint64_t ob = __ballot(occ);
+                uint32_t at0 = 0;
+                if (lane == 0 && ob) at0 = atomicAdd((uint32_t*)(__attribute__((address_space(3))) uint32_t*)&lc[1], (uint32_t)__popcll(ob));
+                const uint32_t at = __builtin_amdgcn_readfirstlane(at0) + rank_below(ob);
+                if (occ) {
+#pragma unroll
+                    for (int w = 0; w <= NW; ++w) lc[kCacheHeaderWords + at * S + w] = ew[w];
+                }
+            }
+            __syncthreads();
+            const uint32_t n_occupied = __builtin_amdgcn_readfirstlane(lc[1]);
+            const unsigned long long listed64 = (listed + 63ull) & ~63ull;
+            const uint32_t parts = leaf_parts(m, listed, leaf_waves);
+            const uint32_t children_per_part = leaf_children_per_part(kb, m, parts);
+            const uint64_t items = listed64 * parts;
+            const bool even = items < (1ull << 28) || own_segment;
+            const uint64_t share_len = even ? ((items + leaf_waves - 1) / leaf_waves + 63) / 64 * 64 : 4096u;
+            const uint32_t dyn_chunk = even ? 0u : 4096u;
+            const uint64_t dyn_first = leaf_waves * share_len;
+            q = WaveQueue{0, 0, dyn_chunk != 0 && items > dyn_first};
+            if (leaf_share * share_len < items) {
+                q.next = leaf_share * share_len;
+                q.end = (q.next + share_len < items) ? q.next + share_len : items;
+            }
+            for (;;) {
+                if (q.next == q.end) {
+                    if (!q.more) break;
+                    BSX_RARE_PARAMS(Pr);
+                    const uint64_t b = dyn_first + grab_chunk(&Pr->ctr->cursor, dyn_chunk, (int)lane);
+                    if (b >= items) { q.more = false; continue; }
+                    q.next = b; q.end = (b + dyn_chunk < items) ? b + dyn_chunk : items;
+                }
+                const uint64_t avail = q.end - q.next;
+                const uint32_t n = avail < 64u ? (uint32_t)avail : 64u;
+                const uint32_t part = (uint32_t)(q.next / listed64);
+                const unsigned long long pbase = q.next - (unsigned long long)part * listed64;
+                const bool lv = lane < n && pbase + lane < listed;
+                uint32_t Sp[NW], Y[NW], tagp = 0;
+#pragma unroll
+                for (int w = 0; w < NW; ++w) { Sp[w] = 0; Y[w] = 0; }
+                if (lv) {
+                    const uint32_t* ent = parents + (pbase + lane) * (NW + 1);
+#pragma unroll
+                    for (int w = 0; w < NW; ++w) Sp[w] = ent[w];
+                    tagp = ent[NW];
+                    net_step<NW, K>(nv, Sp, fm0, fv0, Y, has_fixed);
+                    nexec += part == 0u ? 1u : 0u;
+                }
+                q.next += n;
+                uint32_t hits = 0;
+                for (uint32_t sl = 0; sl < n_occupied; ++sl) {
+                    const uint32_t* e = cbase + sl * S;
+                    const uint32_t tagw = __builtin_amdgcn_readfirstlane(e[NW]);
+                    if ((tagw & kTagMask) == 0) continue;
+                    {
+                        uint32_t d0 = 0;
+#pragma unroll
+                        for (int w = 0; w < NW; ++w) d0 |= (e[w] ^ Sp[w]) & ~added[w];
+                        if (lv && d0 == 0 && part == 0u) {
+                            const uint32_t lam0 = lamtab[(tagw & kTagMask) - 1];
+                            account_fix(tagw, 0u, lam0, 1ll);
+                            account_fix(tagw, 1u, lam0, -1ll);
+                        }
+                        if (tagw & kTagRep) continue;
+                    }
+                    uint32_t d = 0;
+#pragma unroll
+                    for (int w = 0; w < NW; ++w) d |= (e[w] ^ Y[w]) & indep[w];
+                    bool ok = lv && d == 0;
+                    if (!__ballot(ok)) continue;
+                    const uint32_t shift = leaf_free_shift<NW>(Sp, e, dep_lds, n_enum, n_free, kb, m);
+                    ok = ok && shift != kLeafNoChild;
+                    if (!__ballot(ok)) continue;
+                    uint32_t n_hit = leaf_enum_hits<NW>(Sp, e, dep_lds, n_enum, m, part, parts) << (shift & 31u);
+                    n_hit = ok ? n_hit : 0u;
+                    if (n_hit) atomicAdd(&wave_cnt[2u * ((tagw & kTagMask) - 1u)], n_hit);
+                    hits += n_hit;
+                }
+                if (lv) atomicAdd(&wave_cnt[2u * (tagp - 1u) + 1u], children_per_part - hits);
+            }
+        }
+        book_outcomes(book_depth);
     }
     if constexpr (!LOWER) for (;;) {
         const bool input = q.more || q.next < q.end;
@@ -830,90 +962,15 @@
         __builtin_amdgcn_wave_barrier();
     }
 
-    __syncthreads();
-#ifdef BSX_DIAG
-    const unsigned long long dbg_t2 = wall_clock64();
-#endif
-    static_assert(kAccs == 64, "one lane per accumulator");
-    if (wave == 0) {
-        const uint32_t a = lane;
-        const unsigned long long cn = acc_cnt[a];
-        const uint64_t nb = __ballot(cn != 0);
-        if (nb) {
-            unsigned long long at0 = 0;
-            if (!cube && lane == 0) at0 = atomicAdd(&P.ctr->log_cursor, (unsigned long long)__popcll(nb));
-            const unsigned long long at = bcast64(at0, 0) + rank_below(nb);
-            if (cn) {
-                const unsigned long long sl = acc_sl[a];
-                if constexpr (cube) {
-                    Counters* c = P.ctr;
-                    atomicAdd(&c->acc_cnt[a], cn);
-                    atomicAdd(&c->acc_sl[a], sl);
-                    const unsigned long long lo = acc_sl2[a];
-                    const unsigned long long old = atomicAdd(&c->acc_sl2_lo[a], lo);
-                    const unsigned long long up = acc_sl2h[a] + ((old + lo < old) ? 1ull : 0ull);
-                    if (up) atomicAdd(&c->acc_sl2_hi[a], up);
-                    c->acc_len[a] = lamtab[a];
-#pragma unroll
-                    for (int w = 0; w < NW; ++w) c->acc_key[a][w] = keytab[a * NW + w];
-                } else if (at < P.log_cap) {
-                    LogRec r;
-#pragma unroll
-                    for (int w = 0; w < kMaxW32; ++w) r.key[w] = 0;
-#pragma unroll
-                    for (int w = 0; w < NW; ++w) r.key[w] = keytab[a * NW + w];
-                    r.length = lamtab[a]; r.pad = 0; r.count = cn; r.sum_l = sl; r.sum_l2_lo = acc_sl2[a]; r.sum_l2_hi = acc_sl2h[a];
-                    P.log[at] = r;
-                } else {
-                    atomicOr(&P.ctr->log_overflow, 1u);
-                }
-                atomicAdd(&wg_ctr[2], sl + cn * lamtab[a]);
-            }
-        }
-    }
-#ifdef BSX_DIAG
-    if (lane == 0) {
-        atomicAdd(&P.ctr->wave_iters, dbg_iters); atomicAdd(&P.ctr->service_rounds, dbg_fresh);
-        atomicAdd(&P.ctr->diag[0], dbg_fresh_keep); atomicAdd(&P.ctr->diag[1], dbg_pool_in);
-        atomicAdd(&P.ctr->diag[2], dbg_pool_keep); atomicAdd(&P.ctr->diag[3], dbg_merged);
-    }
+    flush_sums(P.ctr + ctr_off);
     if (threadIdx.x == 0) {
-        const unsigned long long dbg_t3 = wall_clock64();
-        atomicAdd(&P.ctr->phase_sum[0], dbg_t1 - dbg_t0); atomicMax(&P.ctr->phase_max[0], dbg_t1 - dbg_t0);
-        atomicAdd(&P.ctr->phase_sum[1], dbg_t2 - dbg_t1); atomicMax(&P.ctr->phase_max[1], dbg_t2 - dbg_t1);
-        atomicAdd(&P.ctr->phase_sum[2], dbg_t3 - dbg_t2); atomicMax(&P.ctr->phase_max[2], dbg_t3 - dbg_t2);
-    }
-#endif
-    {
-        const unsigned long long w_exec = wave_sum((unsigned long long)nexec);
-        if (lane == 0 && w_exec) atomicAdd(&wg_ctr[3], w_exec);
-    }
-    __builtin_amdgcn_fence(__ATOMIC_RELEASE, "workgroup");
-    __builtin_amdgcn_s_barrier();
-    __builtin_amdgcn_fence(__ATOMIC_ACQUIRE, "workgroup");
-    if (threadIdx.x == 0) {
-        if constexpr (cube) {
-            BSX_RARE_PARAMS(Pr);
-            if (Pr->level_out) {
-                const uint32_t listed = lc[2];
-                const uint32_t mine = listed < Pr->near_cap ? listed : (uint32_t)Pr->near_cap;
-                lc[1] = mine ? (uint32_t)atomicAdd(&Pr->level_out->n_entries, (unsigned long long)mine) : 0u;
-                if (listed) atomicAdd(&P.ctr->near_classes, (unsigned long long)listed);
-                if (listed > Pr->near_cap) {
-                    atomicOr(&Pr->level_out->abort, 1u);
-                    atomicOr(&P.ctr->near_overflow, 1u);
-                }
-            }
-        }
-        const unsigned long long ref = wg_ctr[2] + (P.cap_rel_inf ? 0ull : wg_ctr[1] * P.max_t);
-        if (ref) atomicAdd(&P.ctr->steps_ref, ref);
-        if (wg_ctr[3]) atomicAdd(&P.ctr->steps_exec, wg_ctr[3]);
-        if (wg_ctr[0]) atomicAdd(&P.ctr->n_none, wg_ctr[0]);
+        if constexpr (cube) { if (!fused_leaf) note_listed(true); }
+        flush_ctrs(P.ctr + ctr_off);
         if constexpr (cube) atomicMax(&P.ctr->t_last, (unsigned long long)wall_clock64());
     }
     if constexpr (cube) {
         BSX_RARE_PARAMS(Pr);
-        if (Pr->level_out) {
+        if (Pr->level_out && !fused_leaf) {
             __syncthreads();
             const uint32_t listed = lc[2], base = lc[1];
             const uint64_t words = (uint64_t)(listed < Pr->near_cap ? listed : (uint32_t)Pr->near_cap) * (NW + 1);
```
